# fluggo/Canvas

Hardware: AMD Instinct MI355X
Metric: Mpixels/s through 4K f16 RGBA colour-matrix+alpha-over chain; % HBM roofline (higher is better)
Workload: dtype f32

## Files before the change

### canvas_amd/_lib.py

```python
import ctypes as C
import os

from .abi import (box2i, fir_filter, rational, rgba_frame_f16, rgba_frame_f32, v2f, video_frame_source_funcs,
                  video_source)

_HERE = os.path.dirname(os.path.abspath(__file__))
LIB_PATH = os.path.join(_HERE, "libcanvas_hip.so")

CHAIN_MAX_LAYERS = 8
DISPLAY_RGBA8, DISPLAY_ARGB32_PREMUL = 0, 1
FIR_PATH_AUTO, FIR_PATH_PASSES, FIR_PATH_TILED, FIR_PATH_TABLES, FIR_PATH_HV, FIR_PATH_ONE_COLUMN, FIR_PATH_TWO_COLUMNS, FIR_PATH_STRIPS, FIR_PATH_TILES = 0, 1, 2, 4, 16, 32, 64, 128, 256
FIR_KERNEL_NONE, FIR_KERNEL_WINDOW, FIR_KERNEL_HALVE, _FIR_KERNEL_RETIRED_3, FIR_KERNEL_VH, FIR_KERNEL_TILED, _FIR_KERNEL_RETIRED_6, FIR_KERNEL_TWO_PASS, FIR_KERNEL_PASS, FIR_KERNEL_HV, FIR_KERNEL_WINDOW_PAIR, FIR_KERNEL_HALVE_PAIR, FIR_KERNEL_TILE_VH, FIR_KERNEL_UNSHARP = range(14)
ARITH_SEPARATE, ARITH_CONTRACTED = 0, 1
LUT_NONE, LUT_REC709_TO_LINEAR_SCENE, LUT_REC709_TO_LINEAR_DISPLAY, LUT_LINEAR_TO_REC709, LUT_LINEAR_TO_SRGB = -1, 0, 1, 2, 3
KEY_SHOW_MATTE = 1
YCC_PROGRESSIVE, YCC_REC709 = 1, 2


class rgba_f32(C.Structure):
    _fields_ = [("r", C.c_float), ("g", C.c_float), ("b", C.c_float), ("a", C.c_float)]


class rgba_frame_dev(C.Structure):
    _fields_ = [("data", C.c_void_p), ("format", C.c_int), ("full_window", box2i), ("current_window", box2i),
                ("stream", C.c_void_p)]


class chain_job(C.Structure):
    _fields_ = [("out", C.POINTER(rgba_frame_f16)), ("layers", C.POINTER(rgba_frame_f16) * CHAIN_MAX_LAYERS),
                ("nlayers", C.c_int)]


class chroma_key(C.Structure):
    _fields_ = [("key", C.c_float * 3), ("tolerance", C.c_float), ("softness", C.c_float), ("spill", C.c_float),
                ("spill_range", C.c_float), ("flags", C.c_int)]


class coded_image(C.Structure):
    _fields_ = [("data", C.c_void_p * 4), ("stride", C.c_int * 4), ("line_count", C.c_int * 4), ("free_func", C.c_void_p)]


P = C.POINTER
rgba_frame_f16_t = rgba_frame_f16
rgba_frame_f32_t = rgba_frame_f32
_u16p, _f32p, _vp = P(C.c_uint16), P(C.c_float), C.c_void_p
_F16, _F32 = P(rgba_frame_f16), P(rgba_frame_f32)

SIGNATURES = {
    "init_half": (None, []),
    "get_frame_time": (C.c_int64, [P(rational), C.c_int]),
    "get_time_frame": (C.c_int, [P(rational), C.c_int64]),
    "gettime": (C.c_int64, []),
    "video_get_frame_f16": (None, [P(video_source), C.c_int, _F16]),
    "video_get_frame_f32": (None, [P(video_source), C.c_int, _F32]),
    "video_get_frame_f16_gl": (None, [P(video_source), C.c_int, _F16]),
    "video_get_frame_f32_gl": (None, [P(video_source), C.c_int, _F32]),
    "video_get_frame_dev": (None, [P(video_source), C.c_int, P(rgba_frame_dev)]),
    "video_copy_frame_f16": (None, [_F16, _F16]),
    "video_copy_frame_alpha_f32": (None, [_F32, _F32, C.c_float]),
    "video_attenuate_f32": (None, [_F32, C.c_float]),
    "cvs_pulldown23_frames": (C.c_int, [C.c_int, C.c_int, P(C.c_int), P(C.c_int)]),
    "cvs_weave_fields_f16_dev": (C.c_int, [_F16, _F16, _vp]),
    "cvs_field_to_frame_f16_dev": (C.c_int, [_F16, _F16, C.c_int, _vp]),
    "cvs_soften_fields_f16_dev": (C.c_int, [_F16, _F16, _vp]),
    "cvs_interlace_fields_f16_dev": (C.c_int, [_F16, _F16, _F16, _vp]),
    "cvs_pulldown23_add_frames": (C.c_int, [C.c_int, C.c_int, P(C.c_int), P(C.c_int)]),
    "video_mix_cross_f32": (None, [_F32, _F32, _F32, C.c_float]),
    "video_mix_cross_f32_pull": (None, [_F32, P(video_source), C.c_int, P(video_source), C.c_int, C.c_float]),
    "video_mix_over_f32": (None, [_F32, _F32, C.c_float]),
    "video_scale_bilinear_f32": (None, [_F32, v2f, _F32, v2f, v2f]),
    "video_scale_bilinear_f32_pull": (None, [_F32, v2f, P(video_source), C.c_int, P(box2i), v2f, v2f]),
    "video_transfer_rec709_to_linear_scene": (None, [_u16p, _u16p, C.c_size_t]),
    "video_transfer_rec709_to_linear_display": (None, [_u16p, _u16p, C.c_size_t]),
    "video_transfer_linear_to_rec709": (None, [_u16p, _u16p, C.c_size_t]),
    "video_transfer_linear_to_sRGB": (None, [_u16p, _u16p, C.c_size_t]),
    "video_get_gamma45_ramp": (P(C.c_uint8), []),
    "video_color_rgb_to_xyz_sdtv": (None, [_F16]),
    "video_color_xyz_to_srgb": (None, [_F16]),
    "filter_createTriangle": (None, [C.c_float, C.c_float, P(fir_filter)]),
    "filter_createLanczos": (None, [C.c_float, C.c_int, C.c_float, P(fir_filter)]),
    "filter_free": (None, [P(fir_filter)]),
    "video_filter_gain_offset_f16": (None, [_F16, _F16, C.c_float, C.c_float]),
    "video_fill_solid_f16": (None, [_F16, P(box2i), P(rgba_f32)]),
    "video_fill_solid_f32": (None, [_F32, P(box2i), P(rgba_f32)]),
    "workspace_create": (_vp, []),
    "workspace_get_length": (C.c_int, [_vp]),
    "workspace_add_item": (_vp, [_vp, _vp, C.c_int64, C.c_int64, C.c_int64, C.c_int64, _vp]),
    "workspace_get_item": (_vp, [_vp, C.c_int]),
    "workspace_remove_item": (None, [_vp]),
    "workspace_as_video_source": (None, [_vp, P(video_source)]),
    "workspace_free": (None, [_vp]),
    "workspace_get_item_pos": (None, [_vp, P(C.c_int64), P(C.c_int64), P(C.c_int64)]),
    "workspace_get_item_offset": (C.c_int64, [_vp]),
    "workspace_set_item_offset": (None, [_vp, C.c_int64]),
    "workspace_get_item_source": (_vp, [_vp]),
    "workspace_set_item_source": (None, [_vp, _vp]),
    "workspace_get_item_tag": (_vp, [_vp]),
    "workspace_set_item_tag": (None, [_vp, _vp]),
    "workspace_update_item": (None, [_vp, P(C.c_int64), P(C.c_int64), P(C.c_int64), P(C.c_int64), P(_vp), P(_vp)]),
    "cvs_set_arithmetic": (C.c_int, [C.c_int]),
    "cvs_get_arithmetic": (C.c_int, []),
    "cvs_init": (C.c_int, [C.c_int]),
    "cvs_device_count": (C.c_int, []),
    "cvs_current_device": (C.c_int, []),
    "cvs_context_open": (C.c_int, [C.c_int]),
    "cvs_context_count": (C.c_int, []),
    "cvs_context_device": (C.c_int, [C.c_int]),
    "cvs_set_context": (C.c_int, [C.c_int]),
    "cvs_current_context": (C.c_int, []),
    "cvs_frame_owner": (C.c_int, [C.c_int64, C.c_int]),
    "cvs_last_error": (C.c_char_p, []),
    "cvs_clear_last_error": (None, []),
    "cvs_set_log_handler": (None, [C.c_void_p, C.c_void_p]),
    "cvs_device_name": (C.c_char_p, []),
    "cvs_compute_units": (C.c_int, []),
    "cvs_malloc": (_vp, [C.c_size_t]),
    "cvs_free": (None, [_vp]),
    "cvs_graph_begin": (C.c_int, [_vp]),
    "cvs_graph_end": (_vp, [_vp]),
    "cvs_graph_launch": (C.c_int, [_vp, _vp]),
    "cvs_graph_destroy": (None, [_vp]),
    "cvs_mem_info": (C.c_int, [P(C.c_size_t), P(C.c_size_t)]),
    "cvs_pool_malloc": (_vp, [C.c_size_t, _vp]),
    "cvs_pool_free": (None, [_vp, _vp]),
    "cvs_pool_trim": (None, []),
    "cvs_memcpy_h2d": (C.c_int, [_vp, _vp, C.c_size_t, _vp]),
    "cvs_memcpy_d2h": (C.c_int, [_vp, _vp, C.c_size_t, _vp]),
    "cvs_memcpy_d2d": (C.c_int, [_vp, _vp, C.c_size_t, _vp]),
    "cvs_memset": (C.c_int, [_vp, C.c_int, C.c_size_t, _vp]),
    "cvs_stream_create": (_vp, []),
    "cvs_stream_destroy": (None, [_vp]),
    "cvs_stream_sync": (C.c_int, [_vp]),
    "cvs_event_create": (_vp, []),
    "cvs_event_destroy": (None, [_vp]),
    "cvs_event_record": (C.c_int, [_vp, _vp]),
    "cvs_event_sync": (C.c_int, [_vp]),
    "cvs_event_elapsed_ms": (C.c_float, [_vp, _vp]),
    "cvs_lut_device": (_vp, [C.c_int]),
    "cvs_lut_host": (_u16p, [C.c_int]),
    "cvs_lut_install": (C.c_int, [C.c_int, _u16p]),
    "cvs_half_to_float_dev": (C.c_int, [_vp, _vp, C.c_size_t, _vp]),
    "cvs_float_to_half_dev": (C.c_int, [_vp, _vp, C.c_size_t, _vp]),
    "cvs_half_to_float_fast_dev": (C.c_int, [_vp, _vp, C.c_size_t, _vp]),
    "cvs_float_to_half_fast_dev": (C.c_int, [_vp, _vp, C.c_size_t, _vp]),
    "cvs_half_lookup_dev": (C.c_int, [_vp, _vp, _vp, C.c_size_t, _vp]),
    "cvs_frame_f16_to_f32_dev": (C.c_int, [_F32, _F16, _vp]),
    "cvs_frame_f32_to_f16_dev": (C.c_int, [_F16, _F32, _vp]),
    "cvs_copy_frame_f16_dev": (C.c_int, [_F16, _F16, _vp]),
    "cvs_copy_frame_alpha_f32_dev": (C.c_int, [_F32, _F32, C.c_float, _vp]),
    "cvs_mix_cross_f32_dev": (C.c_int, [_F32, _F32, _F32, C.c_float, _vp]),
    "cvs_mix_over_f32_dev": (C.c_int, [_F32, _F32, C.c_float, _vp]),
    "cvs_color_matrix_f16_dev": (C.c_int, [_F16, _f32p, C.c_int, C.c_int, _vp]),
    "cvs_color_matrix_f16_to_dev": (C.c_int, [_F16, _F16, _f32p, C.c_int, C.c_int, _vp]),
    "cvs_gain_offset_f16_dev": (C.c_int, [_F16, _F16, C.c_float, C.c_float, _vp]),
    "cvs_fill_solid_f16_dev": (C.c_int, [_F16, P(box2i), P(rgba_f32), _vp]),
    "cvs_fill_solid_f32_dev": (C.c_int, [_F32, P(box2i), P(rgba_f32), _vp]),
    "cvs_scale_bilinear_f16_dev": (C.c_int, [_F16, v2f, _F16, v2f, v2f, _vp]),
    "cvs_scale_bilinear_f32_dev": (C.c_int, [_F32, v2f, _F32, v2f, v2f, _vp]),
    "cvs_fir_blur_f32_dev": (C.c_int, [_F32, _F32, _f32p, C.c_int, _vp]),
    "coded_image_alloc": (P(coded_image), [P(C.c_int), P(C.c_int), C.c_int]),
    "coded_image_alloc0": (P(coded_image), [P(C.c_int), P(C.c_int), C.c_int]),
    "video_reconstruct_dv": (None, [_F16, P(coded_image)]),
    "video_subsample_dv": (P(coded_image), [_F16]),
    "cvs_reconstruct_dv_dev": (C.c_int, [_F16, P(coded_image), _vp]),
    "cvs_subsample_dv_dev": (C.c_int, [P(coded_image), _F16, C.c_int, _vp]),
    "video_subsample_mpeg2": (P(coded_image), [_F16]),
    "cvs_subsample_mpeg2_dev": (C.c_int, [P(coded_image), _F16, C.c_int, C.c_int, _vp]),
    "video_reconstruct_mpeg2": (None, [_F16, P(coded_image)]),
    "cvs_reconstruct_mpeg2_dev": (C.c_int, [_F16, P(coded_image), C.c_int, C.c_int, C.c_int, _vp]),
    "cvs_frame_to_bytes_dev": (C.c_int, [_vp, _F16, C.c_int, C.c_int, _vp]),
    "video_frame_to_bytes": (C.c_int, [_vp, _F16, C.c_int, C.c_int]),
    "cvs_frame_to_rgba8_intent_dev": (C.c_int, [_vp, _F16, C.c_int, C.c_float, _vp]),
    "video_frame_to_rgba8_intent": (C.c_int, [_vp, _F16, C.c_int, C.c_float]),
    "cvs_fir_blur_f16_dev": (C.c_int, [_F16, _F16, _f32p, C.c_int, _vp]),
    "cvs_unsharp_mask_f32_dev": (C.c_int, [_F32, _F32, _f32p, C.c_int, C.c_float, C.c_float, _vp]),
    "cvs_unsharp_mask_f16_dev": (C.c_int, [_F16, _F16, _f32p, C.c_int, C.c_float, C.c_float, _vp]),
    "cvs_chroma_key_f32_dev": (C.c_int, [_F32, _F32, P(chroma_key), _vp]),
    "cvs_chroma_key_f16_dev": (C.c_int, [_F16, _F16, P(chroma_key), _vp]),
    "cvs_blur_over_f16_dev": (C.c_int, [_F16, _F16, _f32p, C.c_int, P(_F16), C.c_int, _vp]),
    "cvs_resample_lanczos_f32_dev": (C.c_int, [_F32, _F32, C.c_float, C.c_float, C.c_int, _vp]),
    "cvs_resample_lanczos_f16_dev": (C.c_int, [_F16, _F16, C.c_float, C.c_float, C.c_int, _vp]),
    "cvs_blur_lanczos_f16_dev": (C.c_int, [_F16, _F16, _f32p, C.c_int, C.c_float, C.c_float, C.c_int, _vp]),
    "cvs_blur_over_f16_batch_dev": (C.c_int, [P(_F16), P(_F16), _f32p, C.c_int, P(_F16), C.c_int, C.c_int, _vp]),
    "cvs_scale_bilinear_f16_batch_dev": (C.c_int, [P(_F16), v2f, P(_F16), v2f, v2f, C.c_int, _vp]),
    "cvs_scale_bilinear_f32_batch_dev": (C.c_int, [P(_F32), v2f, P(_F32), v2f, v2f, C.c_int, _vp]),
    "cvs_blur_lanczos_f16_batch_dev": (C.c_int, [P(_F16), P(_F16), C.c_int, _f32p, C.c_int, C.c_float, C.c_float, C.c_int, _vp]),
    "cvs_fir_path_override": (None, [C.c_int]),
    "cvs_chain_color_over_f16_dev": (C.c_int, [P(chain_job), C.c_int, _f32p, C.c_int, C.c_int, _vp]),
    "cvs_chain_last_was_fused": (C.c_int, []),
    "cvs_scale_last_was_fused": (C.c_int, []),
    "cvs_fir_last_kernel": (C.c_int, []),
    "cvs_fir_fell_through_count": (C.c_int, []),
    "cvs_chain_last_launch_count": (C.c_int, []),
    "cvs_mix_cross_f16_dev": (C.c_int, [_F16, _F16, _F16, C.c_float, _vp]),
}

HALF_POINTER_GLOBALS = {
    "half_convert_to_float": C.CFUNCTYPE(None, _f32p, _u16p, C.c_int),
    "half_convert_from_float": C.CFUNCTYPE(None, _u16p, _f32p, C.c_int),
    "half_convert_to_float_fast": C.CFUNCTYPE(None, _f32p, _u16p, C.c_int),
    "half_convert_from_float_fast": C.CFUNCTYPE(None, _u16p, _f32p, C.c_int),
    "half_lookup": C.CFUNCTYPE(None, _u16p, _u16p, _u16p, C.c_int),
}

_lib = None


class LibraryMissing(RuntimeError):
    pass


def load():
    global _lib
    if _lib is not None:
        return _lib
    if not os.path.exists(LIB_PATH):
        raise LibraryMissing(
            "%s not found: build it with `python -c 'import __graft_entry__ as g; g.build()'` "
            "(or make -C canvas_amd/csrc).  There is no CPU fallback." % LIB_PATH)
    lib = C.CDLL(LIB_PATH, mode=C.RTLD_GLOBAL)
    for name, (res, args) in SIGNATURES.items():
        fn = getattr(lib, name)
        fn.restype, fn.argtypes = res, args
    _lib = lib
    return lib


def half_pointer(name):
    lib = load()
    addr = C.c_void_p.in_dll(lib, name).value
    return HALF_POINTER_GLOBALS[name](addr) if addr else None


def last_error():
    return load().cvs_last_error().decode()


def check(rc, what="call"):
    if rc != 0:
        raise RuntimeError("%s failed (%d): %s" % (what, rc, last_error()))
```

### canvas_amd/csrc/host/scale.c

```c
#define _GNU_SOURCE
#include "internal.h"
#include <limits.h>
#include <math.h>
#include <stdatomic.h>

static _Atomic int g_fir_path = CVS_FIR_PATH_AUTO;

static _Thread_local int t_scale_fused;
CVS_EXPORT int cvs_scale_last_was_fused(void) { return t_scale_fused; }
static _Thread_local int t_fir_kernel;
CVS_EXPORT int cvs_fir_last_kernel(void) { return t_fir_kernel; }
static _Thread_local int t_fell_through;
CVS_EXPORT int cvs_fir_fell_through_count(void) { return t_fell_through; }
static void fir_launch_fell_through(const char *kernel, int rc) {
    (void)hipGetLastError();
    t_fell_through++;
    cvs_log_warning("%s did not launch (%s): falling back to the next FIR kernel", kernel, hipGetErrorString((hipError_t)rc));
}
CVS_EXPORT void cvs_fir_path_override(int mode) { atomic_store(&g_fir_path, mode & (CVS_FIR_PATH_PASSES | CVS_FIR_PATH_TILED | CVS_FIR_PATH_TABLES | CVS_FIR_PATH_HV | CVS_FIR_PATH_ONE_COLUMN | CVS_FIR_PATH_TWO_COLUMNS | CVS_FIR_PATH_STRIPS | CVS_FIR_PATH_TILES)); }

typedef struct { void *data; box2i full, cur; int half; } any_frame;

static size_t any_bytes(const any_frame *f) { return cvs_box_pixels(&f->full) * (f->half ? sizeof(rgba_f16) : sizeof(rgba_f32)); }

typedef struct { void *frame, *data; box2i *full, *cur; } frame_ref;

static frame_ref frame_of(const void *f, int half) {
    frame_ref r = { (void *)f, NULL, NULL, NULL };
    if (f && half) { rgba_frame_f16 *h = r.frame; r.data = h->data; r.full = &h->full_window; r.cur = &h->current_window; }
    else if (f)    { rgba_frame_f32 *g = r.frame; r.data = g->data; r.full = &g->full_window; r.cur = &g->current_window; }
    return r;
}

static frame_ref frame_at(const void *frames, int i, int half) {
    return frame_of(half ? (const void *)((const rgba_frame_f16 *const *)frames)[i] : (const void *)((const rgba_frame_f32 *const *)frames)[i], half);
}

static any_frame any_of(const frame_ref *f, int half) {
    const any_frame a = { f->data, *f->full, *f->cur, half };
    return a;
}

static bool entry_refused(void *target, const void *source, int half, const char *what, frame_ref *t, frame_ref *src) {
    *t = frame_of(target, half);
    *src = frame_of(source, half);
    if (cvs_enter() != 0) { box2i_set_empty(t->cur); return true; }
    if (!cvs_box_contains(src->full, src->cur)) {
        cvs_set_error("%s: the input's current_window lies outside its buffer", what);
        box2i_set_empty(t->cur);
        return true;
    }
    return false;
}

static void batch_empty_from(const void *targets, int from, int count, int half) {
    for (int i = from; i < count; i++) box2i_set_empty(frame_at(targets, i, half).cur);
}

static bool batch_refused(const void *targets, const void *sources, int count, int half, const char *what) {
    if (!targets || !sources) { cvs_set_error("%s: bad arguments", what); return true; }
    for (int i = 0; i < count; i++)
        if (!frame_at(targets, i, half).frame || !frame_at(sources, i, half).frame) {
            cvs_set_error("%s: frame %d of %d is a null pointer", what, i, count);
            return true;
        }
    for (int i = 0; i < count; i++) {
        const frame_ref src = frame_at(sources, i, half);
        if (!cvs_box_contains(src.full, src.cur)) {
            cvs_set_error("%s: the input's current_window lies outside its buffer (frame %d)", what, i);
            batch_empty_from(targets, 0, count, half);
            return true;
        }
    }
    if (cvs_enter() != 0) { batch_empty_from(targets, 0, count, half); return true; }
    return false;
}

static bool same_box(const box2i *a, const box2i *b) { return memcmp(a, b, sizeof *a) == 0; }

static bool batch_group(cvk_frame_batch *b, const void *targets, const void *sources, int half, int first, int n, size_t tbytes, size_t sbytes,
                        const rgba_frame_f16 *const *overlays, int noverlays) {
    const void *in[CVK_FRAME_BATCH * (1 + CVK_BLUR_MAX_OVER)];
    int nin = 0;
    memset(b, 0, sizeof *b);
    b->n = n;
    for (int i = 0; i < n; i++) {
        b->target[i] = frame_at(targets, first + i, half).data;
        in[nin++] = b->source[i] = frame_at(sources, first + i, half).data;
        for (int l = 0; l < noverlays; l++) in[nin++] = b->over[i][l] = overlays[(size_t)(first + i) * noverlays + l]->data;
    }
    if (n < 2) return false;
    for (int i = 0; i < n; i++) {
        const char *o = b->target[i];
        for (int j = 0; j < nin; j++) { const char *q = in[j]; if (q && o < q + sbytes && q < o + tbytes) return false; }
        for (int j = 0; j < i; j++) { const char *q = b->target[j]; if (o < q + tbytes && q < o + tbytes) return false; }
    }
    return true;
}

static int gather_pass(const any_frame *t, const any_frame *src, const cvk_fir_axis *tab, int axis, int t0, int t1, int lo, int hi, hipStream_t s) {
    if (t1 < t0 || hi < lo) return 0;
    cvk_fir_params fp;
    memset(&fp, 0, sizeof fp);
    fp.target = cvs_view(t->data, &t->full);
    fp.source = cvs_view(src->data, &src->full);
    fp.axis = axis;
    fp.t0 = t0; fp.t1 = t1; fp.lo = lo; fp.hi = hi;
    fp.ntaps = tab->ntaps; fp.tap_src = tab->src; fp.taps = tab->taps; fp.stride = tab->stride;
    fp.in_half = src->half; fp.out_half = t->half;
    return CVK(cvk_fir_gather)(&fp, s);
}

static cvk_fir2d_params fir2d_params(const any_frame *t, const any_frame *src, int tx0, int ty0, int tx1, int ty1,
                                     const cvs_fir_table *h, const cvs_fir_table *v) {
    cvk_fir2d_params fp;
    memset(&fp, 0, sizeof fp);
    fp.target = cvs_view(t->data, &t->full);
    fp.source = cvs_view(src->data, &src->full);
    fp.in_half = src->half; fp.out_half = t->half;
    fp.tx0 = tx0; fp.ty0 = ty0; fp.tx1 = tx1; fp.ty1 = ty1;
    fp.h = h->axis; fp.v = v->axis;
    fp.max_sw = h->max_foot > 0 ? h->max_foot : 1;
    return fp;
}


static int triangle_pass(any_frame *target, float tmin, const any_frame *source, float smin, float factor, int axis, hipStream_t s) {
    const box2i srect = source->cur, trect = target->full;
    const int lo = axis ? (srect.min.y > trect.min.y ? srect.min.y : trect.min.y) : (srect.min.x > trect.min.x ? srect.min.x : trect.min.x);
    const int hi = axis ? (srect.max.y < trect.max.y ? srect.max.y : trect.max.y) : (srect.max.x < trect.max.x ? srect.max.x : trect.max.x);
    const int s0 = axis ? srect.min.x : srect.min.y, s1 = axis ? srect.max.x : srect.max.y;
    const int t0 = axis ? trect.min.x : trect.min.y, t1 = axis ? trect.max.x : trect.max.y;

    cvs_fir_table table;
    int rc = cvs_fir_table_triangle(tmin, smin, factor, s0, s1, t0, t1, axis == 0 || lo <= hi, &table);
    if (rc != 0) return rc;
    const int used_lo = table.used_lo, used_hi = table.used_hi;
    {
        const int o0 = axis ? trect.min.y : trect.min.x, o1 = axis ? trect.max.y : trect.max.x;
        const bool covers = used_hi >= used_lo && hi >= lo && used_lo == t0 && used_hi == t1 && lo == o0 && hi == o1;
        if (!covers && any_bytes(target)) {
            hipError_t e_ = hipMemsetAsync(target->data, 0, any_bytes(target), s);
            if (e_ != hipSuccess) { cvs_fir_table_release(&table, s); cvs_set_error("zero fill: %s", hipGetErrorString(e_)); return -1; }
        }
    }
    if (used_hi >= used_lo && hi >= lo) {
        const size_t first = (size_t)(used_lo - t0);
        cvk_fir_axis from = table.axis;
        from.ntaps += first; from.src += first * (size_t)from.stride; from.taps += first * (size_t)from.stride;
        rc = gather_pass(target, source, &from, axis, used_lo, used_hi, lo, hi, s);
        if (rc == 0) t_fir_kernel = CVS_FIR_KERNEL_PASS;
    }
    cvs_fir_table_release(&table, s);
    if (rc != 0) { cvs_set_error("FIR gather launch failed: %s", hipGetErrorString((hipError_t)rc)); return rc; }
    if (axis) box2i_set(&target->cur, used_lo, lo, used_hi, hi);
    else      box2i_set(&target->cur, lo, used_lo, hi, used_hi);
    return 0;
}

static int triangle_fused_vh(any_frame *target, v2f tp, const any_frame *source, v2f sp, v2f fac, const box2i *mid_full,
                             const cvk_frame_batch *batch, hipStream_t s) {
    const box2i *tf = &target->full, *sc = &source->cur;
    const int lo1 = sc->min.x > mid_full->min.x ? sc->min.x : mid_full->min.x, hi1 = sc->max.x < mid_full->max.x ? sc->max.x : mid_full->max.x;
    cvs_fir_table tv, th = { .pin = -1 };
    if (hi1 < lo1) return 1;
    if (cvs_fir_table_triangle(tp.y, sp.y, fac.y, sc->min.y, sc->max.y, mid_full->min.y, mid_full->max.y, true, &tv) != 0) return -1;
    const int vlo = tv.used_lo, vhi = tv.used_hi;
    int rc = 1;
    if (vhi >= vlo) {
        const int lo2 = vlo > tf->min.y ? vlo : tf->min.y, hi2 = vhi < tf->max.y ? vhi : tf->max.y;
        if (hi2 >= lo2 && cvs_fir_table_triangle(tp.x, sp.x, fac.x, lo1, hi1, tf->min.x, tf->max.x, true, &th) == 0) {
            const int hlo = th.used_lo, hhi = th.used_hi;
            cvk_fir2d_params fp = fir2d_params(target, source, tf->min.x, mid_full->min.y, tf->max.x, hi2, &th, &tv);
            const int pinned = atomic_load(&g_fir_path);
            const bool tiles = hhi >= hlo && !(pinned & CVS_FIR_PATH_STRIPS) &&
                               ((pinned & CVS_FIR_PATH_TILES) ? CVK(cvk_fir_tvh_supported)(&fp)
                                : batch && target->half ? false : CVK(cvk_fir_tvh_preferred)(&fp));
            if (batch && !(hhi >= hlo && (tiles || CVK(cvk_fir_vh_supported)(&fp)))) rc = 2;
            else if (hhi >= hlo && (tiles || CVK(cvk_fir_vh_supported)(&fp))) {
                const bool covers = lo2 == tf->min.y && hi2 == tf->max.y;
                hipError_t e = hipSuccess;
                if (batch) {
                    fp.nframes = batch->n;
                    for (int i = 0; i < batch->n; i++) {
                        fp.frame_source[i] = batch->source[i]; fp.frame_target[i] = batch->target[i];
                        if (!covers && any_bytes(target) && e == hipSuccess) e = hipMemsetAsync(batch->target[i], 0, any_bytes(target), s);
                    }
                } else if (!covers && any_bytes(target)) e = hipMemsetAsync(target->data, 0, any_bytes(target), s);
                int krc = e != hipSuccess ? (int)e : tiles ? CVK(cvk_fir_tvh)(&fp, lo2 - fp.ty0, s) : CVK(cvk_fir_vh)(&fp, lo2 - fp.ty0, cvs_cus(), s);
                if (krc == 0) { box2i_set(&target->cur, hlo, lo2, hhi, hi2); t_fir_kernel = tiles ? CVS_FIR_KERNEL_TILE_VH : CVS_FIR_KERNEL_VH; rc = 0; }
                else { fir_launch_fell_through(tiles ? "k_fir_tile_vh" : "k_fir_vh", krc); rc = 1; }
            }
        }
    }
    cvs_fir_table_release(&tv, s); cvs_fir_table_release(&th, s);
    return rc;
}

static int triangle_fused_hv(any_frame *target, v2f tp, const any_frame *source, v2f sp, v2f fac, const box2i *mid_full, hipStream_t s) {
    const box2i *tf = &target->full, *sc = &source->cur;
    const int lo1 = sc->min.y > mid_full->min.y ? sc->min.y : mid_full->min.y, hi1 = sc->max.y < mid_full->max.y ? sc->max.y : mid_full->max.y;
    cvs_fir_table th, tv = { .pin = -1 };
    if (hi1 < lo1) return 1;
    if (cvs_arith() != CVS_ARITH_SEPARATE) return 1;
    if (cvs_fir_table_triangle(tp.x, sp.x, fac.x, sc->min.x, sc->max.x, mid_full->min.x, mid_full->max.x, true, &th) != 0) return -1;
    const int hlo = th.used_lo, hhi = th.used_hi;
    int rc = 1;
    if (hhi >= hlo) {
        const int lo2 = hlo > tf->min.x ? hlo : tf->min.x, hi2 = hhi < tf->max.x ? hhi : tf->max.x;
        if (hi2 >= lo2 && cvs_fir_table_triangle(tp.y, sp.y, fac.y, lo1, hi1, tf->min.y, tf->max.y, true, &tv) == 0) {
            const int vlo = tv.used_lo, vhi = tv.used_hi;
            cvk_fir2d_params fp = fir2d_params(target, source, mid_full->min.x, tf->min.y, hi2, tf->max.y, &th, &tv);
            if (vhi >= vlo && cvk_fir_hv_supported(&fp)) {
                const bool covers = fp.tx0 == tf->min.x && hi2 == tf->max.x;
                hipError_t e = covers || !any_bytes(target) ? hipSuccess : hipMemsetAsync(target->data, 0, any_bytes(target), s);
                int krc = e != hipSuccess ? (int)e : cvk_fir_hv(&fp, cvs_cus(), s);
                if (krc == 0) { box2i_set(&target->cur, lo2, vlo, hi2, vhi); t_fir_kernel = CVS_FIR_KERNEL_HV; rc = 0; }
                else { fir_launch_fell_through("k_fir_hv", krc); rc = 1; }
            }
        }
    }
    cvs_fir_table_release(&tv, s); cvs_fir_table_release(&th, s);
    return rc;
}

static int scale_core(any_frame *target, v2f tp, const any_frame *source, v2f sp, v2f fac, const cvk_frame_batch *batch, hipStream_t s) {
    t_scale_fused = 0;
    t_fir_kernel = CVS_FIR_KERNEL_NONE;
    if (batch && ((fac.x == 1.0f && tp.x == sp.x) || (fac.y == 1.0f && tp.y == sp.y) || fac.x < fac.y ||
                  (atomic_load(&g_fir_path) & (CVS_FIR_PATH_PASSES | CVS_FIR_PATH_TILED)))) return 2;
    if (fac.x == 1.0f && tp.x == sp.x) return triangle_pass(target, tp.y, source, sp.y, fac.y, 0, s);
    if (fac.y == 1.0f && tp.y == sp.y) return triangle_pass(target, tp.x, source, sp.x, fac.x, 1, s);

    any_frame mid;
    memset(&mid, 0, sizeof mid);
    const box2i *tf = &target->full, *sc = &source->cur;
    const bool x_first = fac.x < fac.y;
    const int fl = cvs_arith() == CVS_ARITH_CONTRACTED;
    if (x_first)
        box2i_set(&mid.full, (int)madd_as(fl, -(tp.x - tf->min.x), fac.x, sp.x), sc->min.y,
                  (int)madd_as(fl, tf->max.x - tp.x, fac.x, sp.x), sc->max.y);
    else
        box2i_set(&mid.full, sc->min.x, (int)madd_as(fl, -(tp.y - tf->min.y), fac.y, sp.y),
                  sc->max.x, (int)madd_as(fl, tf->max.y - tp.y, fac.y, sp.y));
    box2i_intersect(&mid.full, &mid.full, tf);
    mid.cur = mid.full;
    if (!(atomic_load(&g_fir_path) & (CVS_FIR_PATH_PASSES | CVS_FIR_PATH_TILED))) {
        int rc = x_first ? triangle_fused_hv(target, tp, source, sp, fac, &mid.full, s) : triangle_fused_vh(target, tp, source, sp, fac, &mid.full, batch, s);
        if (rc == 0) t_scale_fused = 1;
        if (rc <= 0) return rc;
        if (batch) return 2;
    }
    size_t n = cvs_box_pixels(&mid.full);
    mid.data = cvs_pool_malloc(sizeof(rgba_f32) * (n ? n : 1), s);
    if (!mid.data) return -1;
    int rc;
    if (x_first) { rc = triangle_pass(&mid, tp.x, source, sp.x, fac.x, 1, s); if (rc == 0) rc = triangle_pass(target, tp.y, &mid, sp.y, fac.y, 0, s); }
    else         { rc = triangle_pass(&mid, tp.y, source, sp.y, fac.y, 0, s); if (rc == 0) rc = triangle_pass(target, tp.x, &mid, sp.x, fac.x, 1, s); }
    cvs_pool_free(mid.data, s);
    return rc;
}

static int scale_frame(void *target, v2f tp, const void *source, v2f sp, v2f fac, int half, cvs_stream_t stream, const char *what) {
    frame_ref t, src;
    if (entry_refused(target, source, half, what, &t, &src)) return -1;
    hipStream_t s = cvs_pick_stream(stream);
    if (fac.x == 1.0f && tp.x == sp.x && fac.y == 1.0f && tp.y == sp.y)
        return half ? cvs_copy_frame_f16_dev(target, source, s) : cvs_copy_frame_alpha_f32_dev(target, source, 1.0f, s);
    any_frame tf = any_of(&t, half);
    const any_frame sf = any_of(&src, half);
    int rc = scale_core(&tf, tp, &sf, sp, fac, NULL, s);
    *t.cur = tf.cur;
    if (rc != 0) box2i_set_empty(t.cur);
    return rc;
}

CVS_EXPORT int cvs_scale_bilinear_f32_dev(rgba_frame_f32 *target, v2f tp, const rgba_frame_f32 *source, v2f sp, v2f fac, cvs_stream_t stream) {
    return scale_frame(target, tp, source, sp, fac, 0, stream, "cvs_scale_bilinear_f32_dev");
}

CVS_EXPORT int cvs_scale_bilinear_f16_dev(rgba_frame_f16 *target, v2f tp, const rgba_frame_f16 *source, v2f sp, v2f fac, cvs_stream_t stream) {
    return scale_frame(target, tp, source, sp, fac, 1, stream, "cvs_scale_bilinear_f16_dev");
}

static int scale_batch_frames(const void *targets, v2f tp, const void *sources, v2f sp, v2f fac, int count, int half,
                              cvs_stream_t stream, const char *what) {
    if (count <= 0) return 0;
    if (batch_refused(targets, sources, count, half, what)) return -1;
    hipStream_t s = cvs_pick_stream(stream);
    const size_t px = half ? sizeof(rgba_f16) : sizeof(rgba_f32);
    int rc = 0, done = 0;
    for (int base = 0; count > 1 && rc == 0 && done == base && base < count; base += 64) {
        const int end = count - base < 64 ? count : base + 64;
        const frame_ref t0 = frame_at(targets, base, half), s0 = frame_at(sources, base, half);
        bool uniform = end - base > 1 && !box2i_is_empty(s0.cur) && !box2i_is_empty(t0.full) &&
                       !(fac.x == 1.0f && tp.x == sp.x && fac.y == 1.0f && tp.y == sp.y);
        for (int i = base + 1; uniform && i < end; i++) {
            const frame_ref ti = frame_at(targets, i, half), si = frame_at(sources, i, half);
            uniform = same_box(ti.full, t0.full) && same_box(si.full, s0.full) && same_box(si.cur, s0.cur);
        }
        const size_t tbytes = cvs_box_pixels(t0.full) * px, sbytes = cvs_box_pixels(s0.full) * px;
        while (uniform && rc == 0 && done < end) {
            const int n = end - done < CVK_FRAME_BATCH ? end - done : CVK_FRAME_BATCH;
            cvk_frame_batch b;
            if (!batch_group(&b, targets, sources, half, done, n, tbytes, sbytes, NULL, 0)) break;
            const frame_ref td = frame_at(targets, done, half), sd = frame_at(sources, done, half);
            any_frame t = any_of(&td, half);
            const any_frame src = any_of(&sd, half);
            rc = scale_core(&t, tp, &src, sp, fac, &b, s);
            if (rc == 2) { rc = 0; break; }
            if (rc != 0) break;
            for (int i = 0; i < n; i++) *frame_at(targets, done + i, half).cur = t.cur;
            done += n;
        }
    }
    for (; rc == 0 && done < count; done++) {
        void *t = frame_at(targets, done, half).frame;
        const void *src = frame_at(sources, done, half).frame;
        rc = half ? cvs_scale_bilinear_f16_dev(t, tp, src, sp, fac, stream) : cvs_scale_bilinear_f32_dev(t, tp, src, sp, fac, stream);
    }
    if (rc != 0) batch_empty_from(targets, done, count, half);
    return rc;
}

CVS_EXPORT int cvs_scale_bilinear_f16_batch_dev(rgba_frame_f16 *const *targets, v2f tp, const rgba_frame_f16 *const *sources, v2f sp, v2f fac, int count, cvs_stream_t stream) {
    return scale_batch_frames(targets, tp, sources, sp, fac, count, 1, stream, "cvs_scale_bilinear_f16_batch_dev");
}

CVS_EXPORT int cvs_scale_bilinear_f32_batch_dev(rgba_frame_f32 *const *targets, v2f tp, const rgba_frame_f32 *const *sources, v2f sp, v2f fac, int count, cvs_stream_t stream) {
    return scale_batch_frames(targets, tp, sources, sp, fac, count, 0, stream, "cvs_scale_bilinear_f32_batch_dev");
}

CVS_EXPORT void video_scale_bilinear_f32(rgba_frame_f32 *target, v2f tp, rgba_frame_f32 *source, v2f sp, v2f fac) {
    cvs_bridge br;
    rgba_frame_f32 ft, fs;
    cvs_bridge_open(&br);
    CVS_BRIDGE_FRAME(&br, ft, target, CVS_BRIDGE_UPLOAD);
    CVS_BRIDGE_FRAME(&br, fs, source, CVS_BRIDGE_PRIVATE | (box2i_is_empty(&source->current_window) ? 0 : CVS_BRIDGE_UPLOAD));
    CVS_BRIDGE_CALL(&br, cvs_scale_bilinear_f32_dev, &ft, tp, &fs, sp, fac);
    target->current_window = ft.current_window;
    if (cvs_bridge_close(&br, target->data) != 0) box2i_set_empty(&target->current_window);
}

CVS_EXPORT void video_scale_bilinear_f32_pull(rgba_frame_f32 *target, v2f tp, video_source *source, int frame,
                                              box2i *source_rect, v2f sp, v2f fac) {
    if (fac.x == 0.0f || fac.y == 0.0f) { box2i_set_empty(&target->current_window); return; }
    if (fac.x == 1.0f && fac.y == 1.0f && tp.x == sp.x && tp.y == sp.y) { video_get_frame_f32(source, frame, target); return; }
    const box2i *tf = &target->full_window;
    rgba_frame_f32 tmp;
    box2i_set(&tmp.full_window,
              (int)(sp.x - (tp.x - tf->min.x) / fac.x) - 1, (int)(sp.y - (tp.y - tf->min.y) / fac.y) - 1,
              (int)(sp.x + (tf->max.x - tp.x) / fac.x) + 1, (int)(sp.y + (tf->max.y - tp.y) / fac.y) + 1);
    box2i_intersect(&tmp.full_window, &tmp.full_window, source_rect);
    tmp.current_window = tmp.full_window;
    size_t n = cvs_box_pixels(&tmp.full_window);
    tmp.data = malloc(sizeof(rgba_f32) * (n ? n : 1));
    if (!tmp.data) { box2i_set_empty(&target->current_window); return; }
    video_get_frame_f32(source, frame, &tmp);
    video_scale_bilinear_f32(target, tp, &tmp, sp, fac);
    free(tmp.data);
}


static int fir_two_launches(const any_frame *t, const any_frame *src, const box2i *rect, const cvk_fir_axis *h, const cvk_fir_axis *v, hipStream_t s) {
    const box2i *sw = &src->cur;
    any_frame mid = { NULL, *sw, *sw, 0 };
    box2i_set(&mid.full, rect->min.x, sw->min.y, rect->max.x, sw->max.y);
    mid.data = cvs_pool_malloc(cvs_box_pixels(&mid.full) * sizeof(rgba_f32), s);
    if (!mid.data) return -1;
    int rc = gather_pass(&mid, src, h, 1, rect->min.x, rect->max.x, sw->min.y, sw->max.y, s);
    if (rc == 0) rc = gather_pass(t, &mid, v, 0, rect->min.y, rect->max.y, rect->min.x, rect->max.x, s);
    cvs_pool_free(mid.data, s);
    if (rc != 0) { cvs_set_error("FIR gather launch failed: %s", hipGetErrorString((hipError_t)rc)); return -1; }
    t_fir_kernel = CVS_FIR_KERNEL_TWO_PASS;
    return 0;
}

static int fir2d_launch(const any_frame *t, const any_frame *src, const box2i *rect, const cvs_fir_table *h, const cvs_fir_table *v, hipStream_t s) {
    cvk_fir2d_params fp = fir2d_params(t, src, rect->min.x, rect->min.y, rect->max.x, rect->max.y, h, v);
    fp.max_sh = v->max_foot > 0 ? v->max_foot : 1;
    const int force = atomic_load(&g_fir_path);
    if (force & CVS_FIR_PATH_PASSES) return 1;
    const bool pinned = (force & (CVS_FIR_PATH_TILED | CVS_FIR_PATH_HV)) != 0;
    if (cvs_arith() == CVS_ARITH_SEPARATE && ((force & CVS_FIR_PATH_HV) || !pinned) && cvk_fir_hv_supported(&fp)) {
        int rc = cvk_fir_hv(&fp, cvs_cus(), s);
        if (rc == 0) { t_fir_kernel = CVS_FIR_KERNEL_HV; return 0; }
        fir_launch_fell_through("k_fir_hv", rc);
    }
    if (CVK(cvk_fir2d_lds_bytes)(&fp) > 150 * 1024 || h->axis.stride > 64 || v->axis.stride > 64) return 1;
    int rc = CVK(cvk_fir2d)(&fp, s);
    if (rc != 0) { cvs_set_error("fused FIR launch failed: %s", hipGetErrorString((hipError_t)rc)); return -1; }
    t_fir_kernel = CVS_FIR_KERNEL_TILED;
    return 0;
}

static int fir_pair_launch(const any_frame *t, const any_frame *src, const box2i *rect, cvs_fir_table *h, cvs_fir_table *v, hipStream_t s) {
    int rc = fir2d_launch(t, src, rect, h, v, s);
    if (rc == 1) rc = fir_two_launches(t, src, rect, &h->axis, &v->axis, s);
    cvs_fir_table_release(h, s); cvs_fir_table_release(v, s);
    return rc;
}

static int blur_column_pins(void) {
    const int pin = atomic_load(&g_fir_path);
    return (pin & CVS_FIR_PATH_ONE_COLUMN ? CVK_BLUR_ONE_COLUMN : 0) | (pin & CVS_FIR_PATH_TWO_COLUMNS ? CVK_BLUR_TWO_COLUMNS : 0);
}

static bool blur_has_fast_kernel(const float *taps, int ntaps) {
    bool finite = true;
    for (int k = 0; k < ntaps; k++) finite = finite && isfinite(taps[k]);
    return finite && CVK(cvk_blur_supported)(ntaps, 1) && !(atomic_load(&g_fir_path) & CVS_FIR_PATH_TABLES);
}

static bool halving_sweep(cvk_blur_halve_params *hp, float fx, float fy, int ksize, const float *taps, int ntaps, const any_frame *t, const any_frame *src) {
    if (fx != 0.5f || fy != 0.5f || (atomic_load(&g_fir_path) & CVS_FIR_PATH_TABLES)) return false;
    const box2i *tf = &t->full, *sw = &src->cur;
    fir_filter f = { NULL, 0, 0 };
    filter_createLanczos(0.5f, ksize, 0.0f, &f);
    bool usable = f.coeff && f.center == f.width / 2 && f.width <= 16 && ntaps <= 16 &&
                  tf->min.x > -(1 << 22) && tf->max.x < (1 << 22) && tf->min.y > -(1 << 22) && tf->max.y < (1 << 22);
    for (int k = 0; usable && k < f.width; k++) usable = isfinite(f.coeff[k]);
    for (int k = 0; usable && k < ntaps; k++) usable = isfinite(taps[k]);
    if (usable) {
        memset(hp, 0, sizeof *hp);
        hp->target = cvs_view(t->data, tf);
        hp->source = cvs_view(src->data, &src->full);
        hp->in_half = 1; hp->out_half = 1;
        hp->tx0 = tf->min.x; hp->ty0 = tf->min.y; hp->tx1 = tf->max.x; hp->ty1 = tf->max.y;
        hp->sx0 = sw->min.x; hp->sy0 = sw->min.y; hp->sx1 = sw->max.x; hp->sy1 = sw->max.y;
        hp->ntaps1 = ntaps; hp->ntaps2 = f.width;
        memcpy(hp->taps1, taps, sizeof(float) * (size_t)ntaps);
        memcpy(hp->taps2, f.coeff, sizeof(float) * (size_t)f.width);
        hp->flags = blur_column_pins();
    }
    filter_free(&f);
    return usable;
}

static int halving_launch(const cvk_blur_halve_params *hp, hipStream_t s) {
    int rc = CVK(cvk_blur_halve)(hp, cvs_cus(), s);
    if (rc != 0) { cvs_set_error("blur + halving launch failed: %s", hipGetErrorString((hipError_t)rc)); return -1; }
    t_fir_kernel = CVK(cvk_blur_halve_takes_pairs)(hp) ? CVS_FIR_KERNEL_HALVE_PAIR : CVS_FIR_KERNEL_HALVE;
    return 0;
}

static int blur_fused(const any_frame *t, const any_frame *src, const box2i *win, const float *taps, int ntaps,
                      const void *const *over, int nover, const cvk_frame_batch *batch, hipStream_t s) {
    const box2i *sw = &src->cur;
    if (blur_has_fast_kernel(taps, ntaps)) {
        cvk_blur_params bp;
        memset(&bp, 0, sizeof bp);
        bp.nover = nover;
        for (int l = 0; l < nover; l++) bp.over[l] = over[l];
        bp.target = cvs_view(t->data, &t->full);
        bp.source = cvs_view(src->data, &src->full);
        bp.in_half = src->half; bp.out_half = t->half;
        bp.tx0 = win->min.x; bp.ty0 = win->min.y; bp.tx1 = win->max.x; bp.ty1 = win->max.y;
        bp.sx0 = sw->min.x; bp.sy0 = sw->min.y; bp.sx1 = sw->max.x; bp.sy1 = sw->max.y;
        bp.ntaps = ntaps;
        memcpy(bp.taps, taps, sizeof(float) * (size_t)ntaps);
        if (batch) {
            if (!(ntaps & 1) || ntaps > 31) return 1;
            bp.batch = *batch;
        }
        bp.flags = blur_column_pins();
        int rc = CVK(cvk_blur)(&bp, cvs_cus(), s);
        if (rc != 0) { cvs_set_error("blur launch failed: %s", hipGetErrorString((hipError_t)rc)); return -1; }
        t_fir_kernel = CVK(cvk_blur_takes_pairs)(&bp) ? CVS_FIR_KERNEL_WINDOW_PAIR : CVS_FIR_KERNEL_WINDOW;
        return 0;
    }
    if (nover > 0 || batch) return 1;
    cvs_fir_table h, v;
    if (cvs_fir_table_blur(taps, ntaps, win->min.x, win->max.x, sw->min.x, sw->max.x, CVK_FIR2D_TILE_X, &h) != 0) return -1;
    if (cvs_fir_table_blur(taps, ntaps, win->min.y, win->max.y, sw->min.y, sw->max.y, CVK_FIR2D_TILE_Y, &v) != 0) { cvs_fir_table_release(&h, s); return -1; }
    return fir_pair_launch(t, src, win, &h, &v, s);
}

static int lanczos_fused(const any_frame *t, const any_frame *src, float fx, float fy, int ksize, hipStream_t s) {
    const box2i *tfull = &t->full, *sw = &src->cur;
    const float identity = 1.0f;
    cvk_blur_halve_params hp;
    if (halving_sweep(&hp, fx, fy, ksize, &identity, 1, t, src) && CVK(cvk_blur_supported)(hp.ntaps2, 2)) {
        int rc, kernel;
        if (src->half && t->half && CVK(cvk_blur_halve_takes_pairs)(&hp)) {
            rc = CVK(cvk_blur_halve_pair)(&hp, cvs_cus(), s);
            kernel = CVS_FIR_KERNEL_HALVE_PAIR;
        } else {
            cvk_blur_params bp;
            memset(&bp, 0, sizeof bp);
            bp.target = hp.target; bp.source = hp.source;
            bp.in_half = src->half; bp.out_half = t->half;
            bp.tx0 = hp.tx0; bp.ty0 = hp.ty0; bp.tx1 = hp.tx1; bp.ty1 = hp.ty1;
            bp.sx0 = hp.sx0; bp.sy0 = hp.sy0; bp.sx1 = hp.sx1; bp.sy1 = hp.sy1;
            bp.ntaps = hp.ntaps2; bp.step = 2;
            memcpy(bp.taps, hp.taps2, sizeof(float) * (size_t)hp.ntaps2);
            rc = CVK(cvk_blur)(&bp, cvs_cus(), s);
            kernel = CVS_FIR_KERNEL_WINDOW;
        }
        if (rc != 0) { cvs_set_error("resample launch failed: %s", hipGetErrorString((hipError_t)rc)); return -1; }
        t_fir_kernel = kernel;
        return 0;
    }
    cvs_fir_table h, v;
    if (cvs_fir_table_lanczos(fx, ksize, tfull->min.x, tfull->max.x, sw->min.x, sw->max.x, CVK_FIR2D_TILE_X, &h) != 0) return -1;
    if (cvs_fir_table_lanczos(fy, ksize, tfull->min.y, tfull->max.y, sw->min.y, sw->max.y, CVK_FIR2D_TILE_Y, &v) != 0) { cvs_fir_table_release(&h, s); return -1; }
    return fir_pair_launch(t, src, tfull, &h, &v, s);
}

static int fir_blur(void *target, const void *source, const float *taps, int ntaps, int half, cvs_stream_t stream, const char *what) {
    frame_ref t, src;
    if (entry_refused(target, source, half, what, &t, &src)) return -1;
    if (ntaps < 1 || !taps) { cvs_set_error("blur: need at least one tap"); box2i_set_empty(t.cur); return -1; }
    hipStream_t s = cvs_pick_stream(stream);
    box2i win;
    box2i_intersect(&win, src.cur, t.full);
    *t.cur = win;
    if (box2i_is_empty(&win)) return 0;
    const any_frame tf = any_of(&t, half), sf = any_of(&src, half);
    int rc = blur_fused(&tf, &sf, &win, taps, ntaps, NULL, 0, NULL, s);
    if (rc != 0) box2i_set_empty(t.cur);
    return rc;
}

CVS_EXPORT int cvs_fir_blur_f32_dev(rgba_frame_f32 *target, const rgba_frame_f32 *source, const float *taps, int ntaps, cvs_stream_t stream) {
    return fir_blur(target, source, taps, ntaps, 0, stream, "cvs_fir_blur_f32_dev");
}

CVS_EXPORT int cvs_fir_blur_f16_dev(rgba_frame_f16 *target, const rgba_frame_f16 *source, const float *taps, int ntaps, cvs_stream_t stream) {
    return fir_blur(target, source, taps, ntaps, 1, stream, "cvs_fir_blur_f16_dev");
}

static int unsharp_mask(void *target, const void *source, const float *taps, int ntaps, float amount, float threshold, int half,
                        cvs_stream_t stream, const char *what) {
    frame_ref t, src;
    if (entry_refused(target, source, half, what, &t, &src)) return -1;
    if (ntaps < 1 || !taps) { cvs_set_error("unsharp mask: need at least one tap"); box2i_set_empty(t.cur); return -1; }
    hipStream_t s = cvs_pick_stream(stream);
    box2i win;
    box2i_intersect(&win, src.cur, t.full);
    *t.cur = win;
    const bool fused = blur_has_fast_kernel(taps, ntaps) && CVK(cvk_unsharp_supported)(ntaps);
    t_fir_kernel = fused ? CVS_FIR_KERNEL_UNSHARP : CVS_FIR_KERNEL_NONE;
    if (box2i_is_empty(&win)) return 0;
    const any_frame tf = any_of(&t, half), sf = any_of(&src, half);
    int rc;
    if (fused) {
        cvk_unsharp_params up;
        memset(&up, 0, sizeof up);
        up.target = cvs_view(tf.data, &tf.full);
        up.source = cvs_view(sf.data, &sf.full);
        up.half = half;
        up.tx0 = win.min.x; up.ty0 = win.min.y; up.tx1 = win.max.x; up.ty1 = win.max.y;
        up.sx0 = sf.cur.min.x; up.sy0 = sf.cur.min.y; up.sx1 = sf.cur.max.x; up.sy1 = sf.cur.max.y;
        up.ntaps = ntaps;
        up.amount = amount; up.threshold = threshold;
        memcpy(up.taps, taps, sizeof(float) * (size_t)ntaps);
        rc = CVK(cvk_unsharp)(&up, cvs_cus(), s);
        if (rc != 0) { cvs_set_error("unsharp mask launch failed: %s", hipGetErrorString((hipError_t)rc)); rc = -1; }
    } else {
        any_frame mid = { NULL, win, win, 0 };
        mid.data = cvs_pool_malloc(cvs_box_pixels(&win) * sizeof(rgba_f32), s);
        if (!mid.data) { box2i_set_empty(t.cur); return -1; }
        rc = blur_fused(&mid, &sf, &win, taps, ntaps, NULL, 0, NULL, s);
        if (rc == 0) {
            const cvk_rect r = { win.min.x, win.min.y, win.max.x, win.max.y };
            rc = CVK(cvk_unsharp_combine)(cvs_view(tf.data, &tf.full), cvs_view(sf.data, &sf.full), cvs_view(mid.data, &mid.full), r, half, amount, threshold, s);
            if (rc != 0) { cvs_set_error("unsharp mask launch failed: %s", hipGetErrorString((hipError_t)rc)); rc = -1; }
        }
        cvs_pool_free(mid.data, s);
    }
    if (rc != 0) box2i_set_empty(t.cur);
    return rc;
}

CVS_EXPORT int cvs_unsharp_mask_f32_dev(rgba_frame_f32 *target, const rgba_frame_f32 *source, const float *taps, int ntaps, float amount, float threshold, cvs_stream_t s) {
    return unsharp_mask(target, source, taps, ntaps, amount, threshold, 0, s, "cvs_unsharp_mask_f32_dev");
}

CVS_EXPORT int cvs_unsharp_mask_f16_dev(rgba_frame_f16 *target, const rgba_frame_f16 *source, const float *taps, int ntaps, float amount, float threshold, cvs_stream_t s) {
    return unsharp_mask(target, source, taps, ntaps, amount, threshold, 1, s, "cvs_unsharp_mask_f16_dev");
}

CVS_EXPORT int cvs_blur_over_f16_dev(rgba_frame_f16 *out, const rgba_frame_f16 *source, const float *taps, int ntaps,
                                     const rgba_frame_f16 *const *overlays, int noverlays, cvs_stream_t stream) {
    if (cvs_enter() != 0) { box2i_set_empty(&out->current_window); return -1; }
    CVS_REQUIRE_INSIDE(source, out, "cvs_blur_over_f16_dev");
    if (ntaps < 1 || !taps || noverlays < 0 || (noverlays > 0 && !overlays)) { cvs_set_error("blur+over: bad arguments"); box2i_set_empty(&out->current_window); return -1; }
    if (noverlays == 0) return cvs_fir_blur_f16_dev(out, source, taps, ntaps, stream);
    hipStream_t s = cvs_pick_stream(stream);
    const box2i *full = &out->full_window;
    if (box2i_is_empty(full)) { box2i_set_empty(&out->current_window); return 0; }
    const any_frame o = { out->data, *full, *full, 1 }, src = { (void *)source->data, source->full_window, source->current_window, 1 };
    box2i win;
    box2i_intersect(&win, &source->current_window, full);
    bool whole = noverlays <= CVK_BLUR_MAX_OVER && memcmp(&win, full, sizeof win) == 0;
    const void *bufs[CVK_BLUR_MAX_OVER];
    for (int l = 0; whole && l < noverlays; l++) {
        whole = memcmp(&overlays[l]->full_window, full, sizeof *full) == 0 && memcmp(&overlays[l]->current_window, full, sizeof *full) == 0;
        bufs[l] = overlays[l]->data;
    }
    int rc = 1;
    if (whole && noverlays > 0) rc = blur_fused(&o, &src, &win, taps, ntaps, bufs, noverlays, NULL, s);
    if (rc == 0) { out->current_window = *full; return 0; }
    if (rc < 0) { box2i_set_empty(&out->current_window); return rc; }

    rgba_frame_f32 acc = { cvs_pool_malloc(cvs_box_pixels(full) * sizeof(rgba_f32), s), *full, *full };
    rgba_frame_f32 tmp = { noverlays > 0 ? cvs_pool_malloc(cvs_box_pixels(full) * sizeof(rgba_f32), s) : NULL, *full, *full };
    rc = (acc.data && (tmp.data || noverlays == 0)) ? 0 : -1;
    if (rc == 0) {
        box2i_set_empty(&acc.current_window);
        if (!box2i_is_empty(&win)) {
            const any_frame a = { acc.data, *full, win, 0 };
            acc.current_window = win;
            rc = blur_fused(&a, &src, &win, taps, ntaps, NULL, 0, NULL, s);
        }
    }
    for (int l = 0; rc == 0 && l < noverlays; l++) {
        rc = cvs_frame_f16_to_f32_dev(&tmp, overlays[l], s);
        if (rc == 0) rc = cvs_mix_over_f32_dev(&acc, &tmp, 1.0f, s);
    }
    if (rc == 0) rc = cvs_frame_f32_to_f16_dev(out, &acc, s);
    cvs_pool_free(acc.data, s); cvs_pool_free(tmp.data, s);
    if (rc != 0) box2i_set_empty(&out->current_window);
    return rc;
}

static int resample_lanczos(void *target, const void *source, float fx, float fy, int ksize, int half, cvs_stream_t stream, const char *what) {
    frame_ref t, src;
    if (entry_refused(target, source, half, what, &t, &src)) return -1;
    if (!(fx > 0.0f) || !(fy > 0.0f) || ksize < 1 || box2i_is_empty(src.cur) || box2i_is_empty(t.full)) {
        box2i_set_empty(t.cur);
        return 0;
    }
    hipStream_t s = cvs_pick_stream(stream);
    const any_frame tf = any_of(&t, half), sf = any_of(&src, half);
    int rc = lanczos_fused(&tf, &sf, fx, fy, ksize, s);
    if (rc == 0) *t.cur = *t.full;
    else box2i_set_empty(t.cur);
    return rc;
}

CVS_EXPORT int cvs_resample_lanczos_f32_dev(rgba_frame_f32 *target, const rgba_frame_f32 *source, float fx, float fy, int ksize, cvs_stream_t stream) {
    return resample_lanczos(target, source, fx, fy, ksize, 0, stream, "cvs_resample_lanczos_f32_dev");
}

CVS_EXPORT int cvs_resample_lanczos_f16_dev(rgba_frame_f16 *target, const rgba_frame_f16 *source, float fx, float fy, int ksize, cvs_stream_t stream) {
    return resample_lanczos(target, source, fx, fy, ksize, 1, stream, "cvs_resample_lanczos_f16_dev");
}

CVS_EXPORT int cvs_blur_lanczos_f16_dev(rgba_frame_f16 *target, const rgba_frame_f16 *source, const float *taps, int ntaps,
                                        float fx, float fy, int ksize, cvs_stream_t stream) {
    if (cvs_enter() != 0) { box2i_set_empty(&target->current_window); return -1; }
    CVS_REQUIRE_INSIDE(source, target, "cvs_blur_lanczos_f16_dev");
    if (ntaps < 1 || !taps || !(fx > 0.0f) || !(fy > 0.0f) || ksize < 1) { cvs_set_error("blur+lanczos: bad arguments"); box2i_set_empty(&target->current_window); return -1; }
    if (box2i_is_empty(&source->current_window) || box2i_is_empty(&target->full_window)) { box2i_set_empty(&target->current_window); return 0; }
    hipStream_t s = cvs_pick_stream(stream);
    const box2i *sw = &source->current_window;
    const any_frame tf = { target->data, target->full_window, target->full_window, 1 }, sf = { (void *)source->data, source->full_window, *sw, 1 };
    if (ntaps == 1 && taps[0] == 1.0f) return cvs_resample_lanczos_f16_dev(target, source, fx, fy, ksize, stream);
    cvk_blur_halve_params hp;
    if ((ntaps & 1) && halving_sweep(&hp, fx, fy, ksize, taps, ntaps, &tf, &sf) && CVK(cvk_blur_halve_supported)(ntaps, hp.ntaps2)) {
        const int rc = halving_launch(&hp, s);
        if (rc == 0) target->current_window = target->full_window;
        else box2i_set_empty(&target->current_window);
        return rc;
    }
    any_frame mid = { NULL, *sw, *sw, 0 };
    mid.data = cvs_pool_malloc(cvs_box_pixels(sw) * sizeof(rgba_f32), s);
    if (!mid.data) { box2i_set_empty(&target->current_window); return -1; }
    int rc = blur_fused(&mid, &sf, sw, taps, ntaps, NULL, 0, NULL, s);
    if (rc == 0) rc = lanczos_fused(&tf, &mid, fx, fy, ksize, s);
    if (rc == 0) target->current_window = target->full_window;
    cvs_pool_free(mid.data, s);
    if (rc != 0) box2i_set_empty(&target->current_window);
    return rc;
}

CVS_EXPORT int cvs_blur_over_f16_batch_dev(rgba_frame_f16 *const *outs, const rgba_frame_f16 *const *sources, const float *taps, int ntaps,
                                           const rgba_frame_f16 *const *overlays, int noverlays, int count, cvs_stream_t stream) {
    const char *what = "cvs_blur_over_f16_batch_dev";
    if (count <= 0) return 0;
    if (ntaps < 1 || !taps || noverlays < 0 || (noverlays > 0 && !overlays)) { cvs_set_error("%s: bad arguments", what); return -1; }
    for (int i = 0; i < count; i++)
        for (int l = 0; l < noverlays; l++)
            if (!overlays[(size_t)i * noverlays + l]) { cvs_set_error("%s: layer %d of frame %d is a null pointer", what, l, i); return -1; }
    if (batch_refused(outs, sources, count, 1, what)) return -1;
    hipStream_t s = cvs_pick_stream(stream);
    const box2i *full = &outs[0]->full_window;
    bool uniform = count > 1 && noverlays >= 1 && noverlays <= CVK_BLUR_MAX_OVER && !box2i_is_empty(full) && blur_has_fast_kernel(taps, ntaps) && (ntaps & 1);
    for (int i = 0; uniform && i < count; i++) {
        uniform = same_box(&outs[i]->full_window, full) && same_box(&sources[i]->full_window, &sources[0]->full_window) &&
                  same_box(&sources[i]->current_window, full) && same_box(&sources[0]->full_window, full);
        for (int l = 0; uniform && l < noverlays; l++) {
            const rgba_frame_f16 *ov = overlays[(size_t)i * noverlays + l];
            uniform = same_box(&ov->full_window, full) && same_box(&ov->current_window, full);
        }
    }
    int rc = 0, done = 0;
    const size_t bytes = cvs_box_pixels(full) * sizeof(rgba_f16);
    while (uniform && rc == 0 && done < count) {
        const int n = count - done < CVK_FRAME_BATCH ? count - done : CVK_FRAME_BATCH;
        cvk_frame_batch b;
        if (!batch_group(&b, outs, sources, 1, done, n, bytes, bytes, overlays, noverlays)) break;
        const any_frame t = { b.target[0], *full, *full, 1 }, src = { (void *)b.source[0], sources[done]->full_window, sources[done]->current_window, 1 };
        rc = blur_fused(&t, &src, full, taps, ntaps, b.over[0], noverlays, &b, s);
        if (rc == 1) { rc = 0; break; }
        if (rc == 0) { for (int i = 0; i < n; i++) outs[done + i]->current_window = *full; done += n; }
    }
    for (; rc == 0 && done < count; done++)
        rc = cvs_blur_over_f16_dev(outs[done], sources[done], taps, ntaps, noverlays ? overlays + (size_t)done * noverlays : NULL, noverlays, stream);
    if (rc != 0) batch_empty_from(outs, done, count, 1);
    return rc;
}

CVS_EXPORT int cvs_blur_lanczos_f16_batch_dev(rgba_frame_f16 *const *targets, const rgba_frame_f16 *const *sources, int count,
                                              const float *taps, int ntaps, float fx, float fy, int ksize, cvs_stream_t stream) {
    const char *what = "cvs_blur_lanczos_f16_batch_dev";
    if (count <= 0) return 0;
    if (ntaps < 1 || !taps || !(fx > 0.0f) || !(fy > 0.0f) || ksize < 1) { cvs_set_error("%s: bad arguments", what); return -1; }
    if (batch_refused(targets, sources, count, 1, what)) return -1;
    hipStream_t s = cvs_pick_stream(stream);
    int rc = 0, done = 0;
    const box2i *tf = &targets[0]->full_window, *sw = &sources[0]->current_window;
    bool uniform = count > 1 && (ntaps & 1) && !(ntaps == 1 && taps[0] == 1.0f) && !box2i_is_empty(sw) && !box2i_is_empty(tf);
    for (int i = 1; uniform && i < count; i++)
        uniform = same_box(&targets[i]->full_window, tf) && same_box(&sources[i]->full_window, &sources[0]->full_window) &&
                  same_box(&sources[i]->current_window, sw);
    const any_frame t0 = { targets[0]->data, *tf, *tf, 1 }, s0 = { (void *)sources[0]->data, sources[0]->full_window, *sw, 1 };
    cvk_blur_halve_params hp;
    if (uniform && halving_sweep(&hp, fx, fy, ksize, taps, ntaps, &t0, &s0) && CVK(cvk_blur_halve_supported)(ntaps, hp.ntaps2)) {
        const size_t sbytes = cvs_box_pixels(&sources[0]->full_window) * sizeof(rgba_f16), tbytes = cvs_box_pixels(tf) * sizeof(rgba_f16);
        while (rc == 0 && done < count) {
            const int n = count - done < CVK_FRAME_BATCH ? count - done : CVK_FRAME_BATCH;
            if (!batch_group(&hp.batch, targets, sources, 1, done, n, tbytes, sbytes, NULL, 0)) break;
            hp.target.data = hp.batch.target[0];
            hp.source.data = (void *)hp.batch.source[0];
            if ((rc = halving_launch(&hp, s)) != 0) break;
            for (int i = 0; i < n; i++) targets[done + i]->current_window = targets[done + i]->full_window;
            done += n;
        }
    }
    for (; rc == 0 && done < count; done++)
        rc = cvs_blur_lanczos_f16_dev(targets[done], sources[done], taps, ntaps, fx, fy, ksize, stream);
    if (rc != 0) batch_empty_from(targets, done, count, 1);
    return rc;
}
```

### canvas_amd/csrc/kernels/blur_pair_ops.hip

```cpp
#include <cstdlib>
#include <atomic>
#include "pair_common.hpp"

namespace {

using namespace pairsweep;

template <int NT, int W, int NOV>
__global__ __launch_bounds__(W) void k_blur_pair(cvk_blur_params bp) {
    constexpr int C = NT / 2, D = C & 1, OUTW = 2 * W - 2 * C - 2 * D, PITCH = W + 8;
    static_assert(NT & 1 && NT >= 3 && NT <= 15, "odd tap counts up to 15");
    static_assert(NOV >= 0 && NOV <= CVK_BLUR_MAX_OVER, "layer count");
    __shared__ float4 rowbuf[2][2][PITCH];
    const int lane = threadIdx.x;
    const int xo = bp.tx0 + (int)blockIdx.x * OUTW;
    const int sfirst = xo - C - D;
    const int tcol = xo + 2 * lane;
    const int ta = bp.ty0 + (int)blockIdx.y * bp.rows_per_wg;
    const int tb = min(ta + bp.rows_per_wg - 1, bp.ty1);
    const int ys0 = ta - C;
    const int steps = (tb - ta) + NT;

    float w[NT];
#pragma unroll
    for (int k = 0; k < NT; k++) w[k] = bp.taps[k];

    const int z = (int)blockIdx.z;
    typedef const cvk_blur_params __attribute__((address_space(4))) *kargs_t;
    const kargs_t ka = (kargs_t)__builtin_amdgcn_kernarg_segment_ptr();
    const void *src_data = bp.batch.n ? ka->batch.source[z] : bp.source.data;
    void *dst_data = bp.batch.n ? ka->batch.target[z] : bp.target.data;
    const void *over_data[NOV > 0 ? NOV : 1];
#pragma unroll
    for (int l = 0; l < NOV; l++) over_data[l] = bp.batch.n ? ka->batch.over[z][l] : bp.over[l];

    const size_t srow = (size_t)bp.source.pitch * 8, trow = (size_t)bp.target.pitch * 8;
    const uint32_t soff = (uint32_t)((sfirst + 2 * lane - bp.sx0) * 8);
    const uint32_t toff = 2 * lane < OUTW ? (uint32_t)((tcol - bp.tx0) * 8) : 0x80000000u;
#ifdef CVS_DIAG
    const uint32_t swin = (bp.flags & 0x100) ? 0u : (uint32_t)(bp.sx1 - bp.sx0 + 1) * 8u, trect = (uint32_t)(bp.tx1 - bp.tx0 + 1) * 8u;
    const uint32_t orect = (bp.flags & 0x200) ? 0u : trect, wrect = (bp.flags & 0x400) ? 0u : trect;
#else
    const uint32_t swin = (uint32_t)(bp.sx1 - bp.sx0 + 1) * 8u, trect = (uint32_t)(bp.tx1 - bp.tx0 + 1) * 8u, orect = trect, wrect = trect;
#endif
    const char *swin0 = reinterpret_cast<const char *>(src_data) + (ptrdiff_t)(bp.sx0 - bp.source.fx0) * 8;
    const ptrdiff_t trect0 = (ptrdiff_t)(bp.tx0 - bp.target.fx0) * 8;

    if (lane < PITCH - W) {
#pragma unroll
        for (int b = 0; b < 2; b++)
#pragma unroll
            for (int ph = 0; ph < 2; ph++) rowbuf[b][ph][W + lane] = make_float4(0.f, 0.f, 0.f, 0.f);
    }

    Px ring[NT][2];
#pragma unroll
    for (int k = 0; k < NT; k++) ring[k][0].rg = ring[k][0].ba = ring[k][1].rg = ring[k][1].ba = f32x2{ 0.0f, 0.0f };

    auto fetch_row = [&](int ys, bool wanted) {
        const bool live = wanted && ys >= bp.sy0 && ys <= bp.sy1;
        return load_pair(row_rsrc(swin0, (size_t)((ptrdiff_t)(ys - bp.source.fy0) * (ptrdiff_t)srow), live ? swin : 0u), soff);
    };
    struct Layers { u32x4 v[NOV > 0 ? NOV : 1]; };
    auto fetch_layers = [&](int i) {
        Layers r;
        const bool emits = i >= NT - 1 && i < steps;
        const size_t o = (size_t)((ptrdiff_t)(ta + i - (NT - 1) - bp.target.fy0) * (ptrdiff_t)trow + trect0);
#pragma unroll
        for (int l = 0; l < NOV; l++) r.v[l] = load_pair(row_rsrc(over_data[l], o, emits ? orect : 0u), toff);
        return r;
    };
    u32x4 cur = fetch_row(ys0, true);
    rowbuf[0][0][lane] = widen_px(cur.x, cur.y);
    rowbuf[0][1][lane] = widen_px(cur.z, cur.w);
    cur = fetch_row(ys0 + 1, steps > 1);
    u32x4 nxt = fetch_row(ys0 + 2, steps > 2);
    Layers ov_cur = fetch_layers(0);

    for (int i0 = 0; i0 < steps; i0 += NT) {
        auto step = [&](auto jc) -> bool {
            constexpr int j = decltype(jc)::value;
            const int i = i0 + j;
            if (i >= steps) return false;
            const bool emits = i >= NT - 1;
            const int t = ta + (i - (NT - 1));
            const u32x4 far = fetch_row(ys0 + i + 3, i + 3 < steps);
            const Layers ov_nxt = fetch_layers(i + 1);
            float4 (*buf)[PITCH] = rowbuf[i & 1];
            __syncthreads();
            float4 v[NT + 1];
#pragma unroll
            for (int c = 0; c <= NT; c++) v[c] = buf[(c + D) & 1][lane + ((c + D) >> 1)];
            float4 (*nbuf)[PITCH] = rowbuf[(i + 1) & 1];
            nbuf[0][lane] = widen_px(cur.x, cur.y);
            nbuf[1][lane] = widen_px(cur.z, cur.w);
            cur = nxt;
            nxt = far;
            f32x2 rg0, ba0, rg1, ba1;
#pragma unroll
            for (int k = 0; k < NT; k++) {
                if constexpr (cvs::kContract) {
                    if (k == 0) { rg0 = f32x2{ v[0].x, v[0].y } * w[0]; ba0 = f32x2{ v[0].z, v[0].w } * w[0]; rg1 = f32x2{ v[1].x, v[1].y } * w[0]; ba1 = f32x2{ v[1].z, v[1].w } * w[0]; }
                    else {
                        rg0 = cvs::madd(f32x2{ v[k].x, v[k].y }, w[k], rg0); ba0 = cvs::madd(f32x2{ v[k].z, v[k].w }, w[k], ba0);
                        rg1 = cvs::madd(f32x2{ v[k + 1].x, v[k + 1].y }, w[k], rg1); ba1 = cvs::madd(f32x2{ v[k + 1].z, v[k + 1].w }, w[k], ba1);
                    }
                } else {
                const f32x2 p0 = f32x2{ v[k].x, v[k].y } * w[k], q0 = f32x2{ v[k].z, v[k].w } * w[k];
                const f32x2 p1 = f32x2{ v[k + 1].x, v[k + 1].y } * w[k], q1 = f32x2{ v[k + 1].z, v[k + 1].w } * w[k];
                if (k == 0) { rg0 = p0; ba0 = q0; rg1 = p1; ba1 = q1; }
                else { rg0 = rg0 + p0; ba0 = ba0 + q0; rg1 = rg1 + p1; ba1 = ba1 + q1; }
                }
            }
            ring[j][0].rg = rg0; ring[j][0].ba = ba0;
            ring[j][1].rg = rg1; ring[j][1].ba = ba1;
            if (emits) {
                f32x2 org0, oba0, org1, oba1;
#pragma unroll
                for (int k = 0; k < NT; k++) {
                    const Px &a = ring[(j + 1 + k) % NT][0], &b = ring[(j + 1 + k) % NT][1];
                    if constexpr (cvs::kContract) {
                        if (k == 0) { org0 = a.rg * w[0]; oba0 = a.ba * w[0]; org1 = b.rg * w[0]; oba1 = b.ba * w[0]; }
                        else { org0 = cvs::madd(a.rg, w[k], org0); oba0 = cvs::madd(a.ba, w[k], oba0); org1 = cvs::madd(b.rg, w[k], org1); oba1 = cvs::madd(b.ba, w[k], oba1); }
                    } else {
                    const f32x2 p0 = a.rg * w[k], q0 = a.ba * w[k], p1 = b.rg * w[k], q1 = b.ba * w[k];
                    if (k == 0) { org0 = p0; oba0 = q0; org1 = p1; oba1 = q1; }
                    else { org0 = org0 + p0; oba0 = oba0 + q0; org1 = org1 + p1; oba1 = oba1 + q1; }
                    }
                }
                u32x4 codes;
                if constexpr (NOV > 0) {
                    cvs::px32x2 acc;
                    acc.r = f32x2{ org0.x, org1.x }; acc.g = f32x2{ org0.y, org1.y };
                    acc.b = f32x2{ oba0.x, oba1.x }; acc.a = f32x2{ oba0.y, oba1.y };
#pragma unroll
                    for (int l = 0; l < NOV; l++) acc = cvs::over_pair_uniform(acc, ov_cur.v[l]);
                    codes = cvs::narrow_pair_lean(acc);
                } else {
                    codes = u32x4{ cvs::f2h_rz2(org0.x, org0.y), cvs::f2h_rz2(oba0.x, oba0.y), cvs::f2h_rz2(org1.x, org1.y), cvs::f2h_rz2(oba1.x, oba1.y) };
                }
                __builtin_amdgcn_raw_buffer_store_b128(codes, row_rsrc(dst_data, (size_t)((ptrdiff_t)(t - bp.target.fy0) * (ptrdiff_t)trow + trect0), wrect), (int)toff, 0, 0);
            }
            ov_cur = ov_nxt;
            return true;
        };
        each_slot(step, std::make_integer_sequence<int, NT>{});
    }
}

template <int NT, int W, int NOV>
int launch(cvk_blur_params bp, int cus, hipStream_t s) {
    constexpr int C = NT / 2, D = C & 1, OUTW = 2 * W - 2 * C - 2 * D;
    const int cols = bp.tx1 - bp.tx0 + 1, rows = bp.ty1 - bp.ty0 + 1;
    const int strips = (cols + OUTW - 1) / OUTW;
    static std::atomic<int> cached{ 0 };
    int mine = cached.load(std::memory_order_relaxed);
    if (!mine) {
        mine = resident_per_cu(k_blur_pair<NT, W, NOV>, W);
        const char *e = CVS_DIAG_ENV("CVS_BLUR_PAIR_WGS");
        if (e && atoi(e) > 0) mine = atoi(e);
        cached.store(mine, std::memory_order_relaxed);
    }
    const int nframes = bp.batch.n > 0 ? bp.batch.n : 1;
    if (bp.rows_per_wg <= 0) {
        int segs = (mine * cus) / (strips * nframes);
        if (segs < 1) segs = 1;
        int r = (rows + segs - 1) / segs;
        if (r < NT - 1) r = NT - 1;
        if (r > rows) r = rows;
        bp.rows_per_wg = r;
    }
    dim3 grid((unsigned)strips, (unsigned)((rows + bp.rows_per_wg - 1) / bp.rows_per_wg), (unsigned)nframes);
    hipLaunchKernelGGL((k_blur_pair<NT, W, NOV>), grid, dim3(W), 0, s, bp);
    return (int)hipGetLastError();
}

template <int NT, int W>
int pick_layers(const cvk_blur_params *bp, int cus, hipStream_t s) {
    switch (bp->nover) {
    case 0: return launch<NT, W, 0>(*bp, cus, s);
    case 1: return launch<NT, W, 1>(*bp, cus, s);
    case 2: return launch<NT, W, 2>(*bp, cus, s);
    case 3: return launch<NT, W, 3>(*bp, cus, s);
    case 4: return launch<NT, W, 4>(*bp, cus, s);
    }
    return (int)hipErrorInvalidValue;
}

template <int W>
int pick(const cvk_blur_params *bp, int cus, hipStream_t s) {
    switch (bp->ntaps) {
    case 3: return pick_layers<3, W>(bp, cus, s);
    case 5: return pick_layers<5, W>(bp, cus, s);
    case 7: return pick_layers<7, W>(bp, cus, s);
    case 9: return pick_layers<9, W>(bp, cus, s);
    case 11: return pick_layers<11, W>(bp, cus, s);
    case 13: return pick_layers<13, W>(bp, cus, s);
    }
    return (int)hipErrorInvalidValue;
}

}

extern "C" int cvk_blur_pair_supported(const cvk_blur_params *bp) {
    if (!(bp->in_half && bp->out_half) || (bp->step != 0 && bp->step != 1)) return 0;
    if (!(bp->ntaps & 1) || bp->ntaps < 3 || bp->ntaps > 13) return 0;
    if (bp->nover < 0 || bp->nover > CVK_BLUR_MAX_OVER) return 0;
    const int c = bp->ntaps / 2, d = c & 1;
    if ((bp->source.pitch | bp->target.pitch) & 1) return 0;
    if (((bp->tx0 - bp->target.fx0) | (bp->tx1 - bp->tx0 + 1)) & 1) return 0;
    if (((bp->sx0 - bp->source.fx0) | (bp->sx1 - bp->sx0 + 1) | (bp->tx0 - c - d - bp->sx0)) & 1) return 0;
    if (bp->sx1 < bp->sx0 || bp->sy1 < bp->sy0) return 0;
    const int n = bp->batch.n > 0 ? bp->batch.n : 1;
    if (n > CVK_FRAME_BATCH) return 0;
    for (int z = 0; z < n; z++) {
        const void *src = bp->batch.n ? bp->batch.source[z] : bp->source.data;
        const void *dst = bp->batch.n ? bp->batch.target[z] : bp->target.data;
        if (!aligned16(src) || !aligned16(dst)) return 0;
        for (int l = 0; l < bp->nover; l++)
            if (!aligned16(bp->batch.n ? bp->batch.over[z][l] : bp->over[l])) return 0;
    }
    return 1;
}

extern "C" int cvk_blur_pair(const cvk_blur_params *bp_in, int cus, void *stream) {
    if (bp_in->tx1 < bp_in->tx0 || bp_in->ty1 < bp_in->ty0) return 0;
    if (!cvk_blur_pair_supported(bp_in)) return (int)hipErrorInvalidValue;
    cvk_blur_params bp = *bp_in;
    bp.step = 1;
    bp.flags = 0;
#ifdef CVS_DIAG
    { const char *e = getenv("CVS_BLUR_PAIR_DROP"); if (e) bp.flags = atoi(e) << 8; }
#endif
    return pick<64>(&bp, cus, (hipStream_t)stream);
}
```

### canvas_amd/csrc/kernels/kernels.h

```cpp
#ifndef CVS_KERNELS_H
#define CVS_KERNELS_H

#include <stddef.h>
#include <stdint.h>

#ifdef CVS_DIAG
#include <stdlib.h>
#define CVS_DIAG_ENV(name) getenv(name)
#else
#define CVS_DIAG_ENV(name) ((const char *)0)
#endif

#ifdef CVS_CONTRACT
#define cvk_gain_offset_f16          cvk_gain_offset_f16_fma
#define cvk_mix                      cvk_mix_fma
#define cvk_color_matrix             cvk_color_matrix_fma
#define cvk_chain_color_over         cvk_chain_color_over_fma
#define cvk_chain_cross              cvk_chain_cross_fma
#define cvk_chain_count_reset        cvk_chain_count_reset_fma
#define cvk_chain_count              cvk_chain_count_fma
#define cvk_fir_gather               cvk_fir_gather_fma
#define cvk_fir2d_lds_bytes          cvk_fir2d_lds_bytes_fma
#define cvk_fir2d                    cvk_fir2d_fma
#define cvk_fir_vh_supported         cvk_fir_vh_supported_fma
#define cvk_fir_vh                   cvk_fir_vh_fma
#define cvk_fir_tvh_supported        cvk_fir_tvh_supported_fma
#define cvk_fir_tvh_preferred        cvk_fir_tvh_preferred_fma
#define cvk_fir_tvh                  cvk_fir_tvh_fma
#define cvk_blur_supported           cvk_blur_supported_fma
#define cvk_blur_takes_pairs         cvk_blur_takes_pairs_fma
#define cvk_blur                     cvk_blur_fma
#define cvk_blur_pair_supported      cvk_blur_pair_supported_fma
#define cvk_blur_pair                cvk_blur_pair_fma
#define cvk_blur_halve_pair_supported cvk_blur_halve_pair_supported_fma
#define cvk_blur_halve_pair          cvk_blur_halve_pair_fma
#define cvk_blur_halve_supported     cvk_blur_halve_supported_fma
#define cvk_blur_halve_takes_pairs   cvk_blur_halve_takes_pairs_fma
#define cvk_blur_halve               cvk_blur_halve_fma
#define cvk_unsharp_supported        cvk_unsharp_supported_fma
#define cvk_unsharp                  cvk_unsharp_fma
#define cvk_unsharp_combine          cvk_unsharp_combine_fma
#define cvk_dv_reconstruct           cvk_dv_reconstruct_fma
#define cvk_dv_subsample             cvk_dv_subsample_fma
#endif

#ifdef __cplusplus
extern "C" {
#endif

typedef struct {
    void *data;
    int pitch;
    int fx0, fy0, fx1, fy1;
} cvk_view;

typedef struct { int x0, y0, x1, y1; } cvk_rect;

int cvk_half_to_float(float *out, const uint16_t *in, size_t count, int fast, void *stream);
int cvk_float_to_half(uint16_t *out, const float *in, size_t count, int fast, void *stream);
int cvk_half_lookup(const uint16_t *table, uint16_t *out, const uint16_t *in, size_t count, int cus, void *stream);

int cvk_copy_f16(cvk_view out, cvk_view in, cvk_rect r, void *stream);
int cvk_copy_alpha_f32(cvk_view out, cvk_view in, cvk_rect r, float alpha, void *stream);
int cvk_weave_f16(cvk_view frame, cvk_rect cur, const void *other, cvk_rect other_cur, void *stream);
int cvk_widen(cvk_view out32, cvk_view in16, cvk_rect r, void *stream);
int cvk_narrow(cvk_view out16, cvk_view in32, cvk_rect r, void *stream);
int cvk_fill_f16(cvk_view out, cvk_rect r, const float rgba[4], void *stream);
int cvk_fill_f32(cvk_view out, cvk_rect r, const float rgba[4], void *stream);
int cvk_gain_offset_f16(cvk_view out, cvk_view in, cvk_rect r, float gain, float offset, void *stream);

enum { CVK_MIX_CROSS = 0, CVK_MIX_OVER = 1 };
typedef struct {
    cvk_view out, p, q;
    cvk_rect outer, inner;
    cvk_rect pw, qw;
    int gap_x, gap_y;
    int top_is_p, bottom_is_p, left_is_p, right_is_p;
    float wp, wq;
    int mode;
    int p_in_place;
} cvk_mix_params;
int cvk_mix(const cvk_mix_params *mp, void *stream);

int cvk_color_matrix(cvk_view dst, cvk_view src, cvk_rect r, const float m[9], const uint16_t *pre_lut,
                     const uint16_t *post_lut, int cus, void *stream);

#define CVK_CHAIN_MAX_LAYERS 8
typedef struct {
    void *out;
    const void *layer[CVK_CHAIN_MAX_LAYERS];
    int nlayers;
    int pad;
    uint64_t npixels;
} cvk_chain_job;
int cvk_chain_color_over(const cvk_chain_job *jobs, int njobs, int uniform_layers, const float *m,
                         const uint16_t *pre_lut, const uint16_t *post_lut, int cus, void *stream);

void cvk_chain_count_reset(void);
int cvk_chain_count(void);

int cvk_chain_cross(const cvk_chain_job *jobs, int njobs, float wa, float wb, int cus, void *stream);

typedef struct {
    cvk_view target, source;
    int axis;
    int t0, t1;
    int lo, hi;
    int s0, s1;
    const int *ntaps;
    const int *tap_src;
    const float *taps;
    int stride;
    int in_half, out_half;
} cvk_fir_params;
int cvk_fir_gather(const cvk_fir_params *fp, void *stream);
int cvk_zero_f32(cvk_view v, void *stream);

typedef struct {
    const int *ntaps, *src;
    const float *taps;
    const int *foot;
    int stride;
    int lines;
    int max_taps;
    int wide_foot;
    int max_active;
    int streamable;
    const uint32_t *lrec;
    const uint32_t *pack;
    int pack_width;
    int span_lines[3];
} cvk_fir_axis;
#define CVK_FIR_LREC 32
#define CVK_AXIS_ALIGN(bytes)              (((size_t)(bytes) + 255) & ~(size_t)255)
#define CVK_AXIS_NLINES(lines)             ((size_t)((lines) > 0 ? (lines) : 1))
#define CVK_AXIS_OFF_SRC(lines)            CVK_AXIS_ALIGN(CVK_AXIS_NLINES(lines) * 4)
#define CVK_AXIS_OFF_TAPS(lines, stride)   (CVK_AXIS_OFF_SRC(lines) + CVK_AXIS_ALIGN(CVK_AXIS_NLINES(lines) * (size_t)(stride) * 4))
#define CVK_AXIS_OFF_FOOT(lines, stride)   (CVK_AXIS_OFF_TAPS(lines, stride) + CVK_AXIS_ALIGN(CVK_AXIS_NLINES(lines) * (size_t)(stride) * 4))
#define CVK_FIR_TVH_LINES 16
typedef struct {
    cvk_view target, source;
    int in_half, out_half;
    int tx0, ty0, tx1, ty1;
    cvk_fir_axis h, v;
    int max_sw, max_sh;
    int nframes, pad_;
    const void *frame_source[8];
    void *frame_target[8];
} cvk_fir2d_params;
#define CVK_FIR2D_TILE_X 32
#define CVK_FIR2D_TILE_Y 16
int cvk_fir_hv_supported(const cvk_fir2d_params *fp);
int cvk_fir_hv(const cvk_fir2d_params *fp, int cus, void *stream);
int cvk_fir_vh_supported(const cvk_fir2d_params *fp);
int cvk_fir_vh(const cvk_fir2d_params *fp, int line0, int cus, void *stream);
int cvk_fir_tvh_supported(const cvk_fir2d_params *fp);
int cvk_fir_tvh_preferred(const cvk_fir2d_params *fp);
int cvk_fir_tvh(const cvk_fir2d_params *fp, int line0, void *stream);
size_t cvk_fir2d_lds_bytes(const cvk_fir2d_params *fp);
int cvk_fir2d(const cvk_fir2d_params *fp, void *stream);

#define CVK_FRAME_BATCH 8
#define CVK_BLUR_MAX_OVER 4
typedef struct {
    int n, pad;
    const void *source[CVK_FRAME_BATCH];
    void *target[CVK_FRAME_BATCH];
    const void *over[CVK_FRAME_BATCH][CVK_BLUR_MAX_OVER];
} cvk_frame_batch;

typedef struct {
    cvk_view target, source;
    int in_half, out_half;
    int tx0, ty0, tx1, ty1;
    int sx0, sy0, sx1, sy1;
    int ntaps;
    int rows_per_wg;
    int step;
    float taps[32];
    int nover;
    int flags;
    const void *over[CVK_BLUR_MAX_OVER];
    cvk_frame_batch batch;
} cvk_blur_params;
#define CVK_BLUR_ONE_COLUMN  1
#define CVK_BLUR_TWO_COLUMNS 2
int cvk_blur_supported(int ntaps, int step);
int cvk_blur(const cvk_blur_params *bp, int cus, void *stream);
int cvk_blur_takes_pairs(const cvk_blur_params *bp);
int cvk_blur_pair_supported(const cvk_blur_params *bp);
int cvk_blur_pair(const cvk_blur_params *bp, int cus, void *stream);

typedef struct {
    cvk_view target, source;
    int in_half, out_half;
    int tx0, ty0, tx1, ty1;
    int sx0, sy0, sx1, sy1;
    int ntaps1, ntaps2;
    int rows_per_wg;
    int flags;
    float taps1[16], taps2[16];
    cvk_frame_batch batch;
} cvk_blur_halve_params;
int cvk_blur_halve_supported(int ntaps1, int ntaps2);
int cvk_blur_halve_pair_supported(const cvk_blur_halve_params *bp);
int cvk_blur_halve_pair(const cvk_blur_halve_params *bp, int cus, void *stream);
int cvk_blur_halve_takes_pairs(const cvk_blur_halve_params *bp);
int cvk_blur_halve(const cvk_blur_halve_params *bp, int cus, void *stream);

typedef struct {
    cvk_view target, source;
    int half;
    int tx0, ty0, tx1, ty1;
    int sx0, sy0, sx1, sy1;
    int ntaps;
    int rows_per_wg;
    float amount, threshold;
    float taps[16];
} cvk_unsharp_params;
int cvk_unsharp_supported(int ntaps);
int cvk_unsharp(const cvk_unsharp_params *up, int cus, void *stream);
int cvk_unsharp_combine(cvk_view out, cvk_view src, cvk_view blurred, cvk_rect r, int half, float amount, float threshold, void *stream);

enum { CVK_DISPLAY_RGBA8 = 0, CVK_DISPLAY_ARGB32_PREMUL = 1 };
int cvk_display(void *dst, cvk_view src, cvk_rect r, const uint8_t *table, int mode, int cus, void *stream);

typedef struct { uint8_t *y, *cb, *cr; int sy, scb, scr; } cvk_dv_planes;
typedef struct { float coeff[16]; int width, center; } cvk_dv_taps;
int cvk_dv_reconstruct(cvk_view frame, cvk_rect cur, const cvk_dv_planes *pl, const cvk_dv_taps *tri, const uint16_t *lut, void *stream);
int cvk_dv_subsample(const cvk_dv_planes *pl, cvk_view frame, cvk_rect w, const cvk_dv_taps *tri, const uint16_t *lut, int encode_in_place, void *stream);

int cvk_mpeg2_subsample(const cvk_dv_planes *pl, cvk_view frame, cvk_rect w, int width, int height, const uint16_t *lut, int cus, void *stream);
int cvk_mpeg2_reconstruct(cvk_view frame, cvk_rect w, const cvk_dv_planes *pl, int width, int height, int progressive, const float mat[9],
                          const uint16_t *lut, int cus, void *stream);

int cvk_field_to_frame(cvk_view out, cvk_view in, cvk_rect w, cvk_rect in_cur, int field, int cus, void *stream);
int cvk_soften_fields(cvk_view out, cvk_view in, cvk_rect w, cvk_rect in_cur, int cus, void *stream);
int cvk_interlace_fields(cvk_view out, cvk_view even, cvk_view odd, cvk_rect w, cvk_rect even_cur, cvk_rect odd_cur, int cus, void *stream);

typedef struct {
    float kpb, kpr, tolerance, inv_soft, inv_spill, spill;
    int soft, fade;
    int matte;
} cvk_key_params;
int cvk_chroma_key(const cvk_key_params *kp, cvk_view out, cvk_view in, cvk_rect w, int half, int cus, void *stream);

#ifndef CVS_CONTRACT
int cvk_gain_offset_f16_fma(cvk_view out, cvk_view in, cvk_rect r, float gain, float offset, void *stream);
int cvk_mix_fma(const cvk_mix_params *mp, void *stream);
int cvk_color_matrix_fma(cvk_view dst, cvk_view src, cvk_rect r, const float m[9], const uint16_t *pre_lut, const uint16_t *post_lut, int cus, void *stream);
int cvk_chain_color_over_fma(const cvk_chain_job *jobs, int njobs, int uniform_layers, const float *m, const uint16_t *pre_lut, const uint16_t *post_lut, int cus, void *stream);
int cvk_chain_cross_fma(const cvk_chain_job *jobs, int njobs, float wa, float wb, int cus, void *stream);
void cvk_chain_count_reset_fma(void);
int cvk_chain_count_fma(void);
int cvk_fir_gather_fma(const cvk_fir_params *fp, void *stream);
size_t cvk_fir2d_lds_bytes_fma(const cvk_fir2d_params *fp);
int cvk_fir2d_fma(const cvk_fir2d_params *fp, void *stream);
int cvk_fir_vh_supported_fma(const cvk_fir2d_params *fp);
int cvk_fir_vh_fma(const cvk_fir2d_params *fp, int line0, int cus, void *stream);
int cvk_fir_tvh_supported_fma(const cvk_fir2d_params *fp);
int cvk_fir_tvh_preferred_fma(const cvk_fir2d_params *fp);
int cvk_fir_tvh_fma(const cvk_fir2d_params *fp, int line0, void *stream);
int cvk_blur_supported_fma(int ntaps, int step);
int cvk_blur_takes_pairs_fma(const cvk_blur_params *bp);
int cvk_blur_fma(const cvk_blur_params *bp, int cus, void *stream);
int cvk_blur_pair_supported_fma(const cvk_blur_params *bp);
int cvk_blur_pair_fma(const cvk_blur_params *bp, int cus, void *stream);
int cvk_blur_halve_pair_supported_fma(const cvk_blur_halve_params *bp);
int cvk_blur_halve_pair_fma(const cvk_blur_halve_params *bp, int cus, void *stream);
int cvk_blur_halve_supported_fma(int ntaps1, int ntaps2);
int cvk_blur_halve_takes_pairs_fma(const cvk_blur_halve_params *bp);
int cvk_blur_halve_fma(const cvk_blur_halve_params *bp, int cus, void *stream);
int cvk_unsharp_supported_fma(int ntaps);
int cvk_unsharp_fma(const cvk_unsharp_params *up, int cus, void *stream);
int cvk_unsharp_combine_fma(cvk_view out, cvk_view src, cvk_view blurred, cvk_rect r, int half, float amount, float threshold, void *stream);
int cvk_dv_reconstruct_fma(cvk_view frame, cvk_rect cur, const cvk_dv_planes *pl, const cvk_dv_taps *tri, const uint16_t *lut, void *stream);
int cvk_dv_subsample_fma(const cvk_dv_planes *pl, cvk_view frame, cvk_rect w, const cvk_dv_taps *tri, const uint16_t *lut, int encode_in_place, void *stream);
#endif

#ifdef __cplusplus
}
#endif
#endif
```

### canvas_amd/stream.py

```python
import ctypes as C

import numpy as np

from . import _lib, synth
from .device import DeviceFrame
from .shard import frames_of_rank

NODE_BYTES_PER_PIXEL = 16 + 16 + 40
BYTES_PER_PIXEL = 16 + 40
OVERLAYS = 3


class GraphStream:

    def __init__(self, width, height, ring=4, matrix=None, pre_lut=_lib.LUT_REC709_TO_LINEAR_SCENE,
                 post_lut=_lib.LUT_NONE, taps=None, overlays=OVERLAYS, first_frame=0, frame_step=1, exact_slots=None, donors=None):
        from . import REC709_RGB_TO_YPBPR
        self.lib = _lib.load()
        self.w, self.h, self.ring, self.overlays = width, height, ring, overlays
        self.full = (0, 0, width - 1, height - 1)
        self.matrix = np.ascontiguousarray(REC709_RGB_TO_YPBPR if matrix is None else matrix, np.float32).reshape(9)
        self.pre_lut, self.post_lut = pre_lut, post_lut
        self.taps = np.ascontiguousarray(synth.gaussian_taps(9, 1.5) if taps is None else taps, np.float32)
        self.slots = []
        nd = 0
        for slot in range(ring):
            exact = exact_slots is None or slot < exact_slots or not donors
            frames = []
            for k in range(overlays + 1):
                d = DeviceFrame(self.full, np.uint16)
                if exact:
                    d.upload(synth.layer_pixels(width, height, k, first_frame + slot * frame_step))
                else:
                    src_frame = donors[(2 * nd) % len(donors)] if k == 0 else donors[(2 * nd + 1) % len(donors)]
                    nd += 1
                    _lib.check(self.lib.cvs_memcpy_d2d(d.ptr, src_frame.ptr, d.nbytes, None), "d2d")
                frames.append(d)
            src, over = frames[0], frames[1:]
            refs = (C.POINTER(_lib.rgba_frame_f16_t) * overlays)(*[C.pointer(o.c) for o in over])
            self.slots.append({"src": src, "over": over, "over_refs": refs, "graded": DeviceFrame(self.full, np.uint16),
                               "out": DeviceFrame(self.full, np.uint16)})
        _lib.check(self.lib.cvs_stream_sync(None), "donor copies")
        self._m = self.matrix.ctypes.data_as(C.POINTER(C.c_float))
        self._t = self.taps.ctypes.data_as(C.POINTER(C.c_float))

    @staticmethod
    def host_inputs(width, height, frame, overlays=OVERLAYS):
        return [synth.layer_frame(width, height, k, frame) for k in range(overlays + 1)]

    def render(self, slot, stream=None):
        s, lib = self.slots[slot % self.ring], self.lib
        _lib.check(lib.cvs_color_matrix_f16_to_dev(s["graded"].ref(), s["src"].ref(), self._m, self.pre_lut, self.post_lut, stream), "colour")
        _lib.check(lib.cvs_blur_over_f16_dev(s["out"].ref(), s["graded"].ref(), self._t, len(self.taps), s["over_refs"],
                                             self.overlays, stream), "blur+over")
        return s["out"]

    def render_batch(self, slots, stream=None):
        lib, n = self.lib, len(slots)
        ss = [self.slots[i % self.ring] for i in slots]
        for s in ss:
            _lib.check(lib.cvs_color_matrix_f16_to_dev(s["graded"].ref(), s["src"].ref(), self._m, self.pre_lut, self.post_lut, stream), "colour")
        key = tuple(i % self.ring for i in slots)
        if getattr(self, "_batch_key", None) != key:
            fp = C.POINTER(_lib.rgba_frame_f16_t)
            self._b_out = (fp * n)(*[C.pointer(s["out"].c) for s in ss])
            self._b_src = (fp * n)(*[C.pointer(s["graded"].c) for s in ss])
            self._b_ov = (fp * (n * self.overlays))(*[C.pointer(o.c) for s in ss for o in s["over"]])
            self._batch_key = key
        _lib.check(lib.cvs_blur_over_f16_batch_dev(self._b_out, self._b_src, self._t, len(self.taps), self._b_ov, self.overlays, n, stream), "blur+over batch")
        return [s["out"] for s in ss]

    def run(self, frames_per_rank, rank=0, world=1, stream=None):
        mine = frames_of_rank(rank, world, frames_per_rank)
        for i, _g in enumerate(mine):
            self.render(i, stream)
        return len(mine)
```

### include/canvas_hip.h

```cpp
#ifndef CANVAS_HIP_H
#define CANVAS_HIP_H

#include <stdint.h>
#include <stddef.h>
#include <stdbool.h>

#if defined(__cplusplus)
extern "C" {
#endif

#define CVS_EXPORT __attribute__((visibility("default")))
#define NS_PER_SEC INT64_C(1000000000)


typedef uint16_t half;
#define HALF_COUNT 65536

typedef struct { int32_t n; uint32_t d; } rational;
typedef struct { int32_t x, y; } v2i;
typedef struct { v2i min, max; } box2i;
typedef struct { float x, y; } v2f;
typedef struct { v2f min, max; } box2f;

typedef struct { half r, g, b, a; } rgba_f16;
typedef struct { uint8_t r, g, b, a; } rgba_u8;
typedef struct { float r, g, b, a; } rgba_f32;

typedef struct { rgba_f16 *data; box2i full_window; box2i current_window; } rgba_frame_f16;
typedef struct { rgba_f32 *data; box2i full_window; box2i current_window; } rgba_frame_f32;

enum { CVS_FORMAT_F16 = 1, CVS_FORMAT_F32 = 2 };
typedef struct {
    void *data;
    int format;
    box2i full_window;
    box2i current_window;
    void *stream;
} rgba_frame_dev;

typedef void (*video_get_frame_func)(void *self, int frame_index, rgba_frame_f16 *frame);
typedef void (*video_get_frame_32_func)(void *self, int frame_index, rgba_frame_f32 *frame);
typedef void (*video_get_frame_dev_func)(void *self, int frame_index, rgba_frame_dev *frame);

#define VIDEO_SOURCE_FLAG_DEVICE 0x1

typedef struct {
    int flags;
    video_get_frame_func get_frame;
    video_get_frame_32_func get_frame_32;
    video_get_frame_dev_func get_frame_dev;
} video_frame_source_funcs;

typedef struct { void *obj; video_frame_source_funcs *funcs; } video_source;

typedef struct { float *coeff; int width; int center; } fir_filter;


static inline void v2i_add(v2i *r, const v2i *a, const v2i *b) { r->x = a->x + b->x; r->y = a->y + b->y; }
static inline void v2i_subtract(v2i *r, const v2i *a, const v2i *b) { r->x = a->x - b->x; r->y = a->y - b->y; }

#if !defined(__cplusplus)
static inline int min(int a, int b) { return a < b ? a : b; }
static inline int max(int a, int b) { return a > b ? a : b; }
static inline int clamp(int v, int lo, int hi) { return min(max(v, lo), hi); }
#endif
static inline float minf(float a, float b) { return a < b ? a : b; }
static inline float maxf(float a, float b) { return a > b ? a : b; }
static inline float clampf(float v, float lo, float hi) { return minf(maxf(v, lo), hi); }

static inline void box2i_set(box2i *b, int x0, int y0, int x1, int y1) { b->min.x = x0; b->min.y = y0; b->max.x = x1; b->max.y = y1; }
static inline void box2i_set_empty(box2i *b) { box2i_set(b, 0, 0, -1, -1); }
static inline bool box2i_is_empty(const box2i *b) { return b->max.x < b->min.x || b->max.y < b->min.y; }
static inline void box2i_intersect(box2i *r, const box2i *a, const box2i *b) {
    int x0 = a->min.x > b->min.x ? a->min.x : b->min.x, y0 = a->min.y > b->min.y ? a->min.y : b->min.y;
    int x1 = a->max.x < b->max.x ? a->max.x : b->max.x, y1 = a->max.y < b->max.y ? a->max.y : b->max.y;
    box2i_set(r, x0, y0, x1, y1);
}
static inline void box2i_union(box2i *r, const box2i *a, const box2i *b) {
    int x0 = a->min.x < b->min.x ? a->min.x : b->min.x, y0 = a->min.y < b->min.y ? a->min.y : b->min.y;
    int x1 = a->max.x > b->max.x ? a->max.x : b->max.x, y1 = a->max.y > b->max.y ? a->max.y : b->max.y;
    box2i_set(r, x0, y0, x1, y1);
}
static inline void box2i_normalize(box2i *b) {
    if (b->min.x > b->max.x) { int32_t t = b->min.x - 1; b->min.x = b->max.x + 1; b->max.x = t; }
    if (b->min.y > b->max.y) { int32_t t = b->min.y - 1; b->min.y = b->max.y + 1; b->max.y = t; }
}
static inline void box2i_get_size(const box2i *b, v2i *r) {
    r->x = b->max.x < b->min.x ? 0 : b->max.x - b->min.x + 1;
    r->y = b->max.y < b->min.y ? 0 : b->max.y - b->min.y + 1;
}
static inline rgba_f16 *video_get_pixel_f16(rgba_frame_f16 *f, int x, int y) {
    return &f->data[(ptrdiff_t)(y - f->full_window.min.y) * (f->full_window.max.x - f->full_window.min.x + 1) + x - f->full_window.min.x];
}
static inline rgba_f32 *video_get_pixel_f32(rgba_frame_f32 *f, int x, int y) {
    return &f->data[(ptrdiff_t)(y - f->full_window.min.y) * (f->full_window.max.x - f->full_window.min.x + 1) + x - f->full_window.min.x];
}


CVS_EXPORT void init_half(void);
CVS_EXPORT extern void (*half_convert_from_float)(half *out, const float *in, int count);
CVS_EXPORT extern void (*half_convert_to_float)(float *out, const half *in, int count);
CVS_EXPORT extern void (*half_convert_from_float_fast)(half *out, const float *in, int count);
CVS_EXPORT extern void (*half_convert_to_float_fast)(float *out, const half *in, int count);
CVS_EXPORT extern void (*half_lookup)(const half *table, half *out, const half *in, int count);

static inline void rgba_f32_to_f16(rgba_f16 *out, const rgba_f32 *in, int count) { half_convert_from_float(&out->r, &in->r, count * 4); }
static inline void rgba_f16_to_f32(rgba_f32 *out, const rgba_f16 *in, int count) { half_convert_to_float(&out->r, &in->r, count * 4); }

CVS_EXPORT int64_t get_frame_time(const rational *frame_rate, int frame);
CVS_EXPORT int get_time_frame(const rational *frame_rate, int64_t time);
CVS_EXPORT int64_t gettime(void);

CVS_EXPORT void video_get_frame_f16(video_source *source, int frame_index, rgba_frame_f16 *frame);
CVS_EXPORT void video_get_frame_f32(video_source *source, int frame_index, rgba_frame_f32 *frame);
CVS_EXPORT void video_get_frame_f16_gl(video_source *source, int frame_index, rgba_frame_f16 *frame);
CVS_EXPORT void video_get_frame_f32_gl(video_source *source, int frame_index, rgba_frame_f32 *frame);
CVS_EXPORT void video_get_frame_dev(video_source *source, int frame_index, rgba_frame_dev *frame);

CVS_EXPORT void video_copy_frame_f16(rgba_frame_f16 *out, rgba_frame_f16 *in);
CVS_EXPORT void video_copy_frame_alpha_f32(rgba_frame_f32 *out, rgba_frame_f32 *in, float alpha);
CVS_EXPORT void video_attenuate_f32(rgba_frame_f32 *frame, float alpha);
CVS_EXPORT void video_mix_cross_f32(rgba_frame_f32 *out, rgba_frame_f32 *a, rgba_frame_f32 *b, float mix_b);
CVS_EXPORT void video_mix_cross_f32_pull(rgba_frame_f32 *out, video_source *a, int frame_a, video_source *b, int frame_b, float mix_b);
CVS_EXPORT void video_mix_over_f32(rgba_frame_f32 *out, rgba_frame_f32 *b, float mix_b);

CVS_EXPORT void video_scale_bilinear_f32(rgba_frame_f32 *target, v2f target_point, rgba_frame_f32 *source, v2f source_point, v2f factors);
CVS_EXPORT void video_scale_bilinear_f32_pull(rgba_frame_f32 *target, v2f target_point, video_source *source, int frame,
                                              box2i *source_rect, v2f source_point, v2f factors);

CVS_EXPORT void video_transfer_rec709_to_linear_scene(half *out, const half *in, size_t count);
CVS_EXPORT void video_transfer_rec709_to_linear_display(half *out, const half *in, size_t count);
CVS_EXPORT void video_transfer_linear_to_rec709(half *out, const half *in, size_t count);
CVS_EXPORT void video_transfer_linear_to_sRGB(half *out, const half *in, size_t count);
CVS_EXPORT const uint8_t *video_get_gamma45_ramp(void);

CVS_EXPORT void video_color_rgb_to_xyz_sdtv(rgba_frame_f16 *frame);
CVS_EXPORT void video_color_xyz_to_srgb(rgba_frame_f16 *frame);

CVS_EXPORT void filter_createTriangle(float sub, float offset, fir_filter *filter);
CVS_EXPORT void filter_createLanczos(float sub, int kernel_size, float offset, fir_filter *filter);
CVS_EXPORT void filter_free(fir_filter *filter);

CVS_EXPORT void video_filter_gain_offset_f16(rgba_frame_f16 *out, rgba_frame_f16 *in, float gain, float offset);

CVS_EXPORT void video_fill_solid_f16(rgba_frame_f16 *frame, const box2i *window, const rgba_f32 *color);
CVS_EXPORT void video_fill_solid_f32(rgba_frame_f32 *frame, const box2i *window, const rgba_f32 *color);

typedef struct workspace_t_tag workspace_t;
typedef struct workspace_item_t_tag workspace_item_t;
CVS_EXPORT workspace_t *workspace_create(void);
CVS_EXPORT int workspace_get_length(workspace_t *workspace);
CVS_EXPORT workspace_item_t *workspace_add_item(workspace_t *self, void *source, int64_t x, int64_t width, int64_t offset, int64_t z, void *tag);
CVS_EXPORT workspace_item_t *workspace_get_item(workspace_t *self, int index);
CVS_EXPORT void workspace_remove_item(workspace_item_t *item);
CVS_EXPORT void workspace_as_video_source(workspace_t *workspace, video_source *source);
CVS_EXPORT void workspace_free(workspace_t *workspace);
CVS_EXPORT void workspace_get_item_pos(workspace_item_t *item, int64_t *x, int64_t *width, int64_t *z);
CVS_EXPORT int64_t workspace_get_item_offset(workspace_item_t *item);
CVS_EXPORT void workspace_set_item_offset(workspace_item_t *item, int64_t offset);
CVS_EXPORT void *workspace_get_item_source(workspace_item_t *item);
CVS_EXPORT void workspace_set_item_source(workspace_item_t *item, void *source);
CVS_EXPORT void *workspace_get_item_tag(workspace_item_t *item);
CVS_EXPORT void workspace_set_item_tag(workspace_item_t *item, void *tag);
CVS_EXPORT void workspace_update_item(workspace_item_t *item, int64_t *x, int64_t *width, int64_t *z, int64_t *offset, void **source, void **tag);


typedef void *cvs_stream_t;

enum { CVS_LUT_NONE = -1, CVS_LUT_REC709_TO_LINEAR_SCENE = 0, CVS_LUT_REC709_TO_LINEAR_DISPLAY = 1,
       CVS_LUT_LINEAR_TO_REC709 = 2, CVS_LUT_LINEAR_TO_SRGB = 3, CVS_LUT_COUNT = 4 };

enum { CVS_ARITH_SEPARATE = 0, CVS_ARITH_CONTRACTED = 1 };
CVS_EXPORT int cvs_set_arithmetic(int mode);
CVS_EXPORT int cvs_get_arithmetic(void);

CVS_EXPORT int cvs_init(int device);
CVS_EXPORT int cvs_device_count(void);
CVS_EXPORT int cvs_current_device(void);

CVS_EXPORT int cvs_context_open(int device);
CVS_EXPORT int cvs_context_count(void);
CVS_EXPORT int cvs_context_device(int ctx);
CVS_EXPORT int cvs_set_context(int ctx);
CVS_EXPORT int cvs_current_context(void);
CVS_EXPORT int cvs_frame_owner(int64_t frame_index, int nowners);
CVS_EXPORT const char *cvs_last_error(void);
CVS_EXPORT void cvs_clear_last_error(void);
enum { CVS_LOG_ERROR = 0, CVS_LOG_WARNING = 1, CVS_LOG_INFO = 2 };
typedef void (*cvs_log_func)(const char *domain, int level, const char *message, void *user_data);
CVS_EXPORT void cvs_set_log_handler(cvs_log_func handler, void *user_data);
CVS_EXPORT const char *cvs_device_name(void);
CVS_EXPORT int cvs_compute_units(void);

CVS_EXPORT void *cvs_malloc(size_t bytes);
CVS_EXPORT void cvs_free(void *dev);
typedef void *cvs_graph_t;
CVS_EXPORT int cvs_graph_begin(cvs_stream_t stream);
CVS_EXPORT cvs_graph_t cvs_graph_end(cvs_stream_t stream);
CVS_EXPORT int cvs_graph_launch(cvs_graph_t graph, cvs_stream_t stream);
CVS_EXPORT void cvs_graph_destroy(cvs_graph_t graph);
CVS_EXPORT int cvs_mem_info(size_t *free_bytes, size_t *total_bytes);
CVS_EXPORT void *cvs_pool_malloc(size_t bytes, cvs_stream_t s);
CVS_EXPORT void cvs_pool_free(void *dev, cvs_stream_t s);
CVS_EXPORT void cvs_pool_trim(void);
CVS_EXPORT int cvs_memcpy_h2d(void *dev, const void *host, size_t bytes, cvs_stream_t s);
CVS_EXPORT int cvs_memcpy_d2h(void *host, const void *dev, size_t bytes, cvs_stream_t s);
CVS_EXPORT int cvs_memcpy_d2d(void *dst, const void *src, size_t bytes, cvs_stream_t s);
CVS_EXPORT int cvs_memset(void *dev, int value, size_t bytes, cvs_stream_t s);
CVS_EXPORT cvs_stream_t cvs_stream_create(void);
CVS_EXPORT void cvs_stream_destroy(cvs_stream_t s);
CVS_EXPORT int cvs_stream_sync(cvs_stream_t s);
typedef void *cvs_event_t;
CVS_EXPORT cvs_event_t cvs_event_create(void);
CVS_EXPORT void cvs_event_destroy(cvs_event_t e);
CVS_EXPORT int cvs_event_record(cvs_event_t e, cvs_stream_t s);
CVS_EXPORT int cvs_event_sync(cvs_event_t e);
CVS_EXPORT float cvs_event_elapsed_ms(cvs_event_t start, cvs_event_t stop);

CVS_EXPORT const half *cvs_lut_device(int which);
CVS_EXPORT const half *cvs_lut_host(int which);
CVS_EXPORT int cvs_lut_install(int which, const half *table_host);

CVS_EXPORT int cvs_half_to_float_dev(float *out, const half *in, size_t count, cvs_stream_t s);
CVS_EXPORT int cvs_float_to_half_dev(half *out, const float *in, size_t count, cvs_stream_t s);
CVS_EXPORT int cvs_half_to_float_fast_dev(float *out, const half *in, size_t count, cvs_stream_t s);
CVS_EXPORT int cvs_float_to_half_fast_dev(half *out, const float *in, size_t count, cvs_stream_t s);
CVS_EXPORT int cvs_half_lookup_dev(const half *table_dev, half *out, const half *in, size_t count, cvs_stream_t s);

CVS_EXPORT int cvs_frame_f16_to_f32_dev(rgba_frame_f32 *out, const rgba_frame_f16 *in, cvs_stream_t s);
CVS_EXPORT int cvs_frame_f32_to_f16_dev(rgba_frame_f16 *out, const rgba_frame_f32 *in, cvs_stream_t s);
CVS_EXPORT int cvs_copy_frame_f16_dev(rgba_frame_f16 *out, const rgba_frame_f16 *in, cvs_stream_t s);
CVS_EXPORT int cvs_copy_frame_alpha_f32_dev(rgba_frame_f32 *out, const rgba_frame_f32 *in, float alpha, cvs_stream_t s);
CVS_EXPORT int cvs_mix_cross_f32_dev(rgba_frame_f32 *out, const rgba_frame_f32 *a, const rgba_frame_f32 *b, float mix_b, cvs_stream_t s);
CVS_EXPORT int cvs_mix_over_f32_dev(rgba_frame_f32 *out, const rgba_frame_f32 *b, float mix_b, cvs_stream_t s);
CVS_EXPORT int cvs_color_matrix_f16_dev(rgba_frame_f16 *frame, const float m[9], int pre_lut, int post_lut, cvs_stream_t s);
CVS_EXPORT int cvs_color_matrix_f16_to_dev(rgba_frame_f16 *out, const rgba_frame_f16 *in, const float m[9], int pre_lut, int post_lut, cvs_stream_t s);
CVS_EXPORT int cvs_gain_offset_f16_dev(rgba_frame_f16 *out, const rgba_frame_f16 *in, float gain, float offset, cvs_stream_t s);
CVS_EXPORT int cvs_fill_solid_f16_dev(rgba_frame_f16 *frame, const box2i *window, const rgba_f32 *color, cvs_stream_t s);
CVS_EXPORT int cvs_fill_solid_f32_dev(rgba_frame_f32 *frame, const box2i *window, const rgba_f32 *color, cvs_stream_t s);
CVS_EXPORT int cvs_scale_bilinear_f16_dev(rgba_frame_f16 *target, v2f tp, const rgba_frame_f16 *source, v2f sp, v2f fac, cvs_stream_t stream);
CVS_EXPORT int cvs_scale_bilinear_f32_batch_dev(rgba_frame_f32 *const *targets, v2f target_point, const rgba_frame_f32 *const *sources, v2f source_point,
                                                v2f factors, int count, cvs_stream_t stream);
CVS_EXPORT int cvs_scale_bilinear_f16_batch_dev(rgba_frame_f16 *const *targets, v2f target_point, const rgba_frame_f16 *const *sources, v2f source_point,
                                                v2f factors, int count, cvs_stream_t stream);
CVS_EXPORT int cvs_scale_bilinear_f32_dev(rgba_frame_f32 *target, v2f target_point, const rgba_frame_f32 *source, v2f source_point, v2f factors, cvs_stream_t s);
CVS_EXPORT int cvs_fir_blur_f32_dev(rgba_frame_f32 *target, const rgba_frame_f32 *source, const float *taps_host, int ntaps, cvs_stream_t s);
#define CODED_IMAGE_MAX_PLANES 4
typedef struct {
    void *data[CODED_IMAGE_MAX_PLANES];
    int stride[CODED_IMAGE_MAX_PLANES];
    int line_count[CODED_IMAGE_MAX_PLANES];
    void (*free_func)(void *image);
} coded_image;
CVS_EXPORT coded_image *coded_image_alloc(const int *strides, const int *line_counts, int count);
CVS_EXPORT coded_image *coded_image_alloc0(const int *strides, const int *line_counts, int count);
CVS_EXPORT void video_reconstruct_dv(rgba_frame_f16 *frame, coded_image *planar);
CVS_EXPORT coded_image *video_subsample_dv(rgba_frame_f16 *frame);
CVS_EXPORT int cvs_reconstruct_dv_dev(rgba_frame_f16 *frame, const coded_image *planar, cvs_stream_t stream);
CVS_EXPORT int cvs_subsample_dv_dev(coded_image *planar, rgba_frame_f16 *frame, int encode_input_in_place, cvs_stream_t stream);
CVS_EXPORT coded_image *video_subsample_mpeg2(rgba_frame_f16 *frame);
CVS_EXPORT int cvs_subsample_mpeg2_dev(coded_image *planar, const rgba_frame_f16 *frame, int width, int height, cvs_stream_t stream);
enum { CVS_YCC_PROGRESSIVE = 1, CVS_YCC_REC709 = 2 };
CVS_EXPORT int cvs_reconstruct_mpeg2_dev(rgba_frame_f16 *frame, const coded_image *planar, int width, int height, int flags, cvs_stream_t stream);
CVS_EXPORT void video_reconstruct_mpeg2(rgba_frame_f16 *frame, coded_image *planar);

CVS_EXPORT int cvs_pulldown23_frames(int offset, int frame_index, int *first, int *second);
CVS_EXPORT int cvs_weave_fields_f16_dev(rgba_frame_f16 *frame, const rgba_frame_f16 *other, cvs_stream_t stream);

CVS_EXPORT int cvs_field_to_frame_f16_dev(rgba_frame_f16 *out, const rgba_frame_f16 *in, int field, cvs_stream_t stream);
CVS_EXPORT int cvs_soften_fields_f16_dev(rgba_frame_f16 *out, const rgba_frame_f16 *in, cvs_stream_t stream);
CVS_EXPORT int cvs_interlace_fields_f16_dev(rgba_frame_f16 *out, const rgba_frame_f16 *even, const rgba_frame_f16 *odd, cvs_stream_t stream);
CVS_EXPORT int cvs_pulldown23_add_frames(int offset, int frame_index, int *even_source, int *odd_source);

enum { CVS_DISPLAY_RGBA8 = 0, CVS_DISPLAY_ARGB32_PREMUL = 1 };
CVS_EXPORT int cvs_frame_to_bytes_dev(void *dst_dev, const rgba_frame_f16 *frame, int pre_lut, int mode, cvs_stream_t stream);
CVS_EXPORT int video_frame_to_bytes(void *dst_host, const rgba_frame_f16 *host_frame, int pre_lut, int mode);
CVS_EXPORT int cvs_frame_to_rgba8_intent_dev(void *dst_dev, const rgba_frame_f16 *frame, int pre_lut, float rendering_intent, cvs_stream_t stream);
CVS_EXPORT int video_frame_to_rgba8_intent(void *dst_host, const rgba_frame_f16 *host_frame, int pre_lut, float rendering_intent);

CVS_EXPORT int cvs_fir_blur_f16_dev(rgba_frame_f16 *target, const rgba_frame_f16 *source, const float *taps, int ntaps, cvs_stream_t stream);
CVS_EXPORT int cvs_unsharp_mask_f32_dev(rgba_frame_f32 *target, const rgba_frame_f32 *source, const float *taps, int ntaps, float amount, float threshold, cvs_stream_t s);
CVS_EXPORT int cvs_unsharp_mask_f16_dev(rgba_frame_f16 *target, const rgba_frame_f16 *source, const float *taps, int ntaps, float amount, float threshold, cvs_stream_t s);
enum { CVS_KEY_SHOW_MATTE = 1 };
typedef struct cvs_chroma_key {
    float key[3];
    float tolerance;
    float softness;
    float spill;
    float spill_range;
    int   flags;
} cvs_chroma_key;
CVS_EXPORT int cvs_chroma_key_f32_dev(rgba_frame_f32 *target, const rgba_frame_f32 *source, const cvs_chroma_key *key, cvs_stream_t s);
CVS_EXPORT int cvs_chroma_key_f16_dev(rgba_frame_f16 *target, const rgba_frame_f16 *source, const cvs_chroma_key *key, cvs_stream_t s);
CVS_EXPORT int cvs_blur_over_f16_dev(rgba_frame_f16 *out, const rgba_frame_f16 *source, const float *taps, int ntaps,
                                     const rgba_frame_f16 *const *overlays, int noverlays, cvs_stream_t stream);
CVS_EXPORT int cvs_resample_lanczos_f32_dev(rgba_frame_f32 *target, const rgba_frame_f32 *source, float factor_x, float factor_y, int kernel_size, cvs_stream_t s);
CVS_EXPORT int cvs_resample_lanczos_f16_dev(rgba_frame_f16 *target, const rgba_frame_f16 *source, float factor_x, float factor_y, int kernel_size, cvs_stream_t s);
CVS_EXPORT int cvs_blur_lanczos_f16_dev(rgba_frame_f16 *target, const rgba_frame_f16 *source, const float *taps_host, int ntaps,
                                        float factor_x, float factor_y, int kernel_size, cvs_stream_t s);
CVS_EXPORT int cvs_blur_over_f16_batch_dev(rgba_frame_f16 *const *outs, const rgba_frame_f16 *const *sources, const float *taps, int ntaps,
                                           const rgba_frame_f16 *const *overlays, int noverlays, int count, cvs_stream_t stream);
CVS_EXPORT int cvs_blur_lanczos_f16_batch_dev(rgba_frame_f16 *const *targets, const rgba_frame_f16 *const *sources, int count,
                                              const float *taps_host, int ntaps, float fx, float fy, int ksize, cvs_stream_t stream);

enum { CVS_FIR_PATH_AUTO = 0, CVS_FIR_PATH_PASSES = 1 , CVS_FIR_PATH_TILED = 2, CVS_FIR_PATH_TABLES = 4 ,
       CVS_FIR_PATH_HV = 16 ,
       CVS_FIR_PATH_ONE_COLUMN = 32 ,
       CVS_FIR_PATH_TWO_COLUMNS = 64 ,
       CVS_FIR_PATH_STRIPS = 128 ,
       CVS_FIR_PATH_TILES = 256  };
CVS_EXPORT void cvs_fir_path_override(int mode);
enum { CVS_FIR_KERNEL_NONE = 0,
       CVS_FIR_KERNEL_WINDOW = 1,
       CVS_FIR_KERNEL_HALVE = 2,
       CVS_FIR_KERNEL_VH = 4,
       CVS_FIR_KERNEL_TILED = 5,
       CVS_FIR_KERNEL_RETIRED_6 = 6,
       CVS_FIR_KERNEL_TWO_PASS = 7,
       CVS_FIR_KERNEL_PASS = 8,
       CVS_FIR_KERNEL_HV = 9,
       CVS_FIR_KERNEL_WINDOW_PAIR = 10,
       CVS_FIR_KERNEL_HALVE_PAIR = 11,
       CVS_FIR_KERNEL_TILE_VH = 12,
       CVS_FIR_KERNEL_UNSHARP = 13 };
CVS_EXPORT int cvs_fir_last_kernel(void);
CVS_EXPORT int cvs_fir_fell_through_count(void);

#define CVS_CHAIN_MAX_LAYERS 8
typedef struct {
    rgba_frame_f16 *out;
    const rgba_frame_f16 *layers[CVS_CHAIN_MAX_LAYERS];
    int nlayers;
} cvs_chain_job;
CVS_EXPORT int cvs_chain_color_over_f16_dev(const cvs_chain_job *jobs, int njobs, const float m[9],
                                            int pre_lut, int post_lut, cvs_stream_t s);
CVS_EXPORT int cvs_chain_last_was_fused(void);
CVS_EXPORT int cvs_scale_last_was_fused(void);
CVS_EXPORT int cvs_chain_last_launch_count(void);
CVS_EXPORT int cvs_mix_cross_f16_dev(rgba_frame_f16 *out, const rgba_frame_f16 *a, const rgba_frame_f16 *b, float mix_b, cvs_stream_t stream);

#if defined(__cplusplus)
}
#endif
#endif
```

Baseline: 257,200.

## Fuse colour-matrix grading into the blur+over pair kernel

Adds a fused colour-matrix + vertical/horizontal blur + alpha-over kernel that applies LUTs and the 3x3 matrix while loading source rows. The blur sweep body moves into a shared header so the plain and graded variants reuse it. The stream pipeline now calls the fused entry point and no longer allocates an intermediate graded frame. This removes one full-frame write and read of the intermediate through HBM, at the cost of extra ALU and LUT lookups inside the blur loop. Unsupported shapes fall back to the old two-kernel path through a pooled temporary.

```diff
diff --git a/canvas_amd/_lib.py b/canvas_amd/_lib.py
--- a/canvas_amd/_lib.py
+++ b/canvas_amd/_lib.py
@@ -182,6 +182,9 @@
     "cvs_resample_lanczos_f16_dev": (C.c_int, [_F16, _F16, C.c_float, C.c_float, C.c_int, _vp]),
     "cvs_blur_lanczos_f16_dev": (C.c_int, [_F16, _F16, _f32p, C.c_int, C.c_float, C.c_float, C.c_int, _vp]),
     "cvs_blur_over_f16_batch_dev": (C.c_int, [P(_F16), P(_F16), _f32p, C.c_int, P(_F16), C.c_int, C.c_int, _vp]),
+    "cvs_color_blur_over_f16_dev": (C.c_int, [_F16, _F16, _f32p, C.c_int, P(_F16), C.c_int, _f32p, C.c_int, C.c_int, _vp]),
+    "cvs_color_blur_over_f16_batch_dev": (C.c_int, [P(_F16), P(_F16), _f32p, C.c_int, P(_F16), C.c_int, C.c_int, _f32p, C.c_int, C.c_int, _vp]),
+    "cvs_color_blur_last_was_fused": (C.c_int, []),
     "cvs_scale_bilinear_f16_batch_dev": (C.c_int, [P(_F16), v2f, P(_F16), v2f, v2f, C.c_int, _vp]),
     "cvs_scale_bilinear_f32_batch_dev": (C.c_int, [P(_F32), v2f, P(_F32), v2f, v2f, C.c_int, _vp]),
     "cvs_blur_lanczos_f16_batch_dev": (C.c_int, [P(_F16), P(_F16), C.c_int, _f32p, C.c_int, C.c_float, C.c_float, C.c_int, _vp]),
diff --git a/canvas_amd/csrc/host/scale.c b/canvas_amd/csrc/host/scale.c
--- a/canvas_amd/csrc/host/scale.c
+++ b/canvas_amd/csrc/host/scale.c
@@ -713,6 +713,125 @@
     return rc;
 }
 
+
+static _Thread_local int t_color_blur_fused = -1;
+CVS_EXPORT int cvs_color_blur_last_was_fused(void) { return t_color_blur_fused; }
+
+static bool bytes_overlap(const void *a, size_t na, const void *b, size_t nb) {
+    const uintptr_t x = (uintptr_t)a, y = (uintptr_t)b;
+    return x < y + nb && y < x + na;
+}
+
+static int color_blur_fused(const any_frame *t, const any_frame *src, const box2i *win, const float m[9], const half *pre, const half *post,
+                            const float *taps, int ntaps, const void *const *over, int nover, const cvk_frame_batch *batch, hipStream_t s) {
+    if (!blur_has_fast_kernel(taps, ntaps) || ntaps > 31) return 1;
+    cvk_blur_params bp;
+    memset(&bp, 0, sizeof bp);
+    bp.nover = nover;
+    for (int l = 0; l < nover; l++) bp.over[l] = over[l];
+    bp.target = cvs_view(t->data, &t->full);
+    bp.source = cvs_view(src->data, &src->full);
+    bp.in_half = bp.out_half = 1;
+    bp.tx0 = win->min.x; bp.ty0 = win->min.y; bp.tx1 = win->max.x; bp.ty1 = win->max.y;
+    bp.sx0 = src->cur.min.x; bp.sy0 = src->cur.min.y; bp.sx1 = src->cur.max.x; bp.sy1 = src->cur.max.y;
+    bp.ntaps = ntaps;
+    memcpy(bp.taps, taps, sizeof(float) * (size_t)ntaps);
+    if (batch) bp.batch = *batch;
+    bp.flags = blur_column_pins();
+    if (!CVK(cvk_grade_blur_pair_supported)(&bp, (const uint16_t *)pre, (const uint16_t *)post)) return 1;
+    const int n = batch ? batch->n : 1;
+    for (int i = 0; i < n; i++)
+        for (int j = 0; j < n; j++)
+            if (bytes_overlap(batch ? batch->target[i] : t->data, any_bytes(t), batch ? batch->source[j] : src->data, any_bytes(src))) return 1;
+    int rc = CVK(cvk_grade_blur_pair)(&bp, m, (const uint16_t *)pre, (const uint16_t *)post, cvs_cus(), s);
+    if (rc != 0) { cvs_set_error("colour + blur launch failed: %s", hipGetErrorString((hipError_t)rc)); return -1; }
+    t_fir_kernel = CVS_FIR_KERNEL_WINDOW_PAIR;
+    return 0;
+}
+
+CVS_EXPORT int cvs_color_blur_over_f16_dev(rgba_frame_f16 *out, const rgba_frame_f16 *source, const float *taps, int ntaps,
+                                           const rgba_frame_f16 *const *overlays, int noverlays, const float m[9], int pre_lut, int post_lut,
+                                           cvs_stream_t stream) {
+    if (cvs_enter() != 0) { box2i_set_empty(&out->current_window); return -1; }
+    CVS_REQUIRE_INSIDE(source, out, "cvs_color_blur_over_f16_dev");
+    if (ntaps < 1 || !taps || !m || noverlays < 0 || (noverlays > 0 && !overlays)) { cvs_set_error("colour+blur+over: bad arguments"); box2i_set_empty(&out->current_window); return -1; }
+    const half *pre = cvs_lut_dev_or_null(pre_lut), *post = cvs_lut_dev_or_null(post_lut);
+    if ((pre_lut != CVS_LUT_NONE && !pre) || (post_lut != CVS_LUT_NONE && !post)) { box2i_set_empty(&out->current_window); return -1; }
+    hipStream_t s = cvs_pick_stream(stream);
+    const box2i *full = &out->full_window;
+    box2i win;
+    box2i_intersect(&win, &source->current_window, full);
+    bool whole = !box2i_is_empty(&win) && noverlays <= CVK_BLUR_MAX_OVER && (noverlays == 0 || same_box(&win, full));
+    const void *bufs[CVK_BLUR_MAX_OVER];
+    for (int l = 0; whole && l < noverlays; l++) {
+        whole = same_box(&overlays[l]->full_window, full) && same_box(&overlays[l]->current_window, full);
+        bufs[l] = overlays[l]->data;
+    }
+    if (whole) {
+        const any_frame o = { out->data, *full, *full, 1 }, src = { (void *)source->data, source->full_window, source->current_window, 1 };
+        const int rc = color_blur_fused(&o, &src, &win, m, pre, post, taps, ntaps, bufs, noverlays, NULL, s);
+        if (rc == 0) { out->current_window = win; t_color_blur_fused = 1; return 0; }
+        if (rc < 0) { box2i_set_empty(&out->current_window); return rc; }
+    }
+    t_color_blur_fused = 0;
+    rgba_frame_f16 graded = { NULL, source->full_window, source->full_window };
+    const size_t n = cvs_box_pixels(&graded.full_window);
+    if (n) {
+        graded.data = cvs_pool_malloc(n * sizeof(rgba_f16), s);
+        if (!graded.data) { box2i_set_empty(&out->current_window); return -1; }
+    }
+    int rc = cvs_color_matrix_f16_to_dev(&graded, source, m, pre_lut, post_lut, stream);
+    if (rc == 0) rc = cvs_blur_over_f16_dev(out, &graded, taps, ntaps, overlays, noverlays, stream);
+    else box2i_set_empty(&out->current_window);
+    cvs_pool_free(graded.data, s);
+    return rc;
+}
+
+CVS_EXPORT int cvs_color_blur_over_f16_batch_dev(rgba_frame_f16 *const *outs, const rgba_frame_f16 *const *sources, const float *taps, int ntaps,
+                                                 const rgba_frame_f16 *const *overlays, int noverlays, int count, const float m[9], int pre_lut,
+                                                 int post_lut, cvs_stream_t stream) {
+    const char *what = "cvs_color_blur_over_f16_batch_dev";
+    if (count <= 0) return 0;
+    if (ntaps < 1 || !taps || !m || noverlays < 0 || (noverlays > 0 && !overlays)) { cvs_set_error("%s: bad arguments", what); return -1; }
+    for (int i = 0; i < count; i++)
+        for (int l = 0; l < noverlays; l++)
+            if (!overlays[(size_t)i * noverlays + l]) { cvs_set_error("%s: layer %d of frame %d is a null pointer", what, l, i); return -1; }
+    if (batch_refused(outs, sources, count, 1, what)) return -1;
+    if (cvs_enter() != 0) { batch_empty_from(outs, 0, count, 1); return -1; }
+    const half *pre = cvs_lut_dev_or_null(pre_lut), *post = cvs_lut_dev_or_null(post_lut);
+    if ((pre_lut != CVS_LUT_NONE && !pre) || (post_lut != CVS_LUT_NONE && !post)) { batch_empty_from(outs, 0, count, 1); return -1; }
+    hipStream_t s = cvs_pick_stream(stream);
+    const box2i *full = &outs[0]->full_window;
+    bool uniform = count > 1 && noverlays >= 1 && noverlays <= CVK_BLUR_MAX_OVER && !box2i_is_empty(full) && (ntaps & 1);
+    for (int i = 0; uniform && i < count; i++) {
+        uniform = same_box(&outs[i]->full_window, full) && same_box(&sources[i]->full_window, &sources[0]->full_window) &&
+                  same_box(&sources[i]->current_window, full) && same_box(&sources[0]->full_window, full);
+        for (int l = 0; uniform && l < noverlays; l++) {
+            const rgba_frame_f16 *ov = overlays[(size_t)i * noverlays + l];
+            uniform = same_box(&ov->full_window, full) && same_box(&ov->current_window, full);
+        }
+    }
+    int rc = 0, done = 0, all_fused = 1;
+    const size_t bytes = cvs_box_pixels(full) * sizeof(rgba_f16);
+    while (uniform && rc == 0 && done < count) {
+        const int n = count - done < CVK_FRAME_BATCH ? count - done : CVK_FRAME_BATCH;
+        cvk_frame_batch b;
+        if (!batch_group(&b, outs, sources, 1, done, n, bytes, bytes, overlays, noverlays)) break;
+        const any_frame t = { b.target[0], *full, *full, 1 }, src = { (void *)b.source[0], sources[done]->full_window, sources[done]->current_window, 1 };
+        rc = color_blur_fused(&t, &src, full, m, pre, post, taps, ntaps, b.over[0], noverlays, &b, s);
+        if (rc == 1) { rc = 0; break; }
+        if (rc == 0) { for (int i = 0; i < n; i++) outs[done + i]->current_window = *full; done += n; }
+    }
+    for (; rc == 0 && done < count; done++) {
+        rc = cvs_color_blur_over_f16_dev(outs[done], sources[done], taps, ntaps, noverlays ? overlays + (size_t)done * noverlays : NULL, noverlays,
+                                         m, pre_lut, post_lut, stream);
+        if (t_color_blur_fused != 1) all_fused = 0;
+    }
+    if (rc != 0) batch_empty_from(outs, done, count, 1);
+    else t_color_blur_fused = all_fused;
+    return rc;
+}
+
 CVS_EXPORT int cvs_blur_lanczos_f16_batch_dev(rgba_frame_f16 *const *targets, const rgba_frame_f16 *const *sources, int count,
                                               const float *taps, int ntaps, float fx, float fy, int ksize, cvs_stream_t stream) {
     const char *what = "cvs_blur_lanczos_f16_batch_dev";
diff --git a/canvas_amd/csrc/kernels/blur_pair_ops.hip b/canvas_amd/csrc/kernels/blur_pair_ops.hip
--- a/canvas_amd/csrc/kernels/blur_pair_ops.hip
+++ b/canvas_amd/csrc/kernels/blur_pair_ops.hip
@@ -1,6 +1,6 @@
 #include <cstdlib>
 #include <atomic>
-#include "pair_common.hpp"
+#include "blur_pair_sweep.hpp"
 
 namespace {
 
@@ -8,18 +8,10 @@
 
 template <int NT, int W, int NOV>
 __global__ __launch_bounds__(W) void k_blur_pair(cvk_blur_params bp) {
-    constexpr int C = NT / 2, D = C & 1, OUTW = 2 * W - 2 * C - 2 * D, PITCH = W + 8;
     static_assert(NT & 1 && NT >= 3 && NT <= 15, "odd tap counts up to 15");
     static_assert(NOV >= 0 && NOV <= CVK_BLUR_MAX_OVER, "layer count");
-    __shared__ float4 rowbuf[2][2][PITCH];
+    __shared__ float4 rowbuf[2][2][StripGeometry<NT, W>::PITCH];
     const int lane = threadIdx.x;
-    const int xo = bp.tx0 + (int)blockIdx.x * OUTW;
-    const int sfirst = xo - C - D;
-    const int tcol = xo + 2 * lane;
-    const int ta = bp.ty0 + (int)blockIdx.y * bp.rows_per_wg;
-    const int tb = min(ta + bp.rows_per_wg - 1, bp.ty1);
-    const int ys0 = ta - C;
-    const int steps = (tb - ta) + NT;
 
     float w[NT];
 #pragma unroll
@@ -34,123 +26,12 @@
 #pragma unroll
     for (int l = 0; l < NOV; l++) over_data[l] = bp.batch.n ? ka->batch.over[z][l] : bp.over[l];
 
-    const size_t srow = (size_t)bp.source.pitch * 8, trow = (size_t)bp.target.pitch * 8;
-    const uint32_t soff = (uint32_t)((sfirst + 2 * lane - bp.sx0) * 8);
-    const uint32_t toff = 2 * lane < OUTW ? (uint32_t)((tcol - bp.tx0) * 8) : 0x80000000u;
-#ifdef CVS_DIAG
-    const uint32_t swin = (bp.flags & 0x100) ? 0u : (uint32_t)(bp.sx1 - bp.sx0 + 1) * 8u, trect = (uint32_t)(bp.tx1 - bp.tx0 + 1) * 8u;
-    const uint32_t orect = (bp.flags & 0x200) ? 0u : trect, wrect = (bp.flags & 0x400) ? 0u : trect;
-#else
-    const uint32_t swin = (uint32_t)(bp.sx1 - bp.sx0 + 1) * 8u, trect = (uint32_t)(bp.tx1 - bp.tx0 + 1) * 8u, orect = trect, wrect = trect;
-#endif
-    const char *swin0 = reinterpret_cast<const char *>(src_data) + (ptrdiff_t)(bp.sx0 - bp.source.fx0) * 8;
-    const ptrdiff_t trect0 = (ptrdiff_t)(bp.tx0 - bp.target.fx0) * 8;
-
-    if (lane < PITCH - W) {
-#pragma unroll
-        for (int b = 0; b < 2; b++)
-#pragma unroll
-            for (int ph = 0; ph < 2; ph++) rowbuf[b][ph][W + lane] = make_float4(0.f, 0.f, 0.f, 0.f);
-    }
-
-    Px ring[NT][2];
-#pragma unroll
-    for (int k = 0; k < NT; k++) ring[k][0].rg = ring[k][0].ba = ring[k][1].rg = ring[k][1].ba = f32x2{ 0.0f, 0.0f };
-
-    auto fetch_row = [&](int ys, bool wanted) {
-        const bool live = wanted && ys >= bp.sy0 && ys <= bp.sy1;
-        return load_pair(row_rsrc(swin0, (size_t)((ptrdiff_t)(ys - bp.source.fy0) * (ptrdiff_t)srow), live ? swin : 0u), soff);
-    };
-    struct Layers { u32x4 v[NOV > 0 ? NOV : 1]; };
-    auto fetch_layers = [&](int i) {
-        Layers r;
-        const bool emits = i >= NT - 1 && i < steps;
-        const size_t o = (size_t)((ptrdiff_t)(ta + i - (NT - 1) - bp.target.fy0) * (ptrdiff_t)trow + trect0);
-#pragma unroll
-        for (int l = 0; l < NOV; l++) r.v[l] = load_pair(row_rsrc(over_data[l], o, emits ? orect : 0u), toff);
-        return r;
-    };
-    u32x4 cur = fetch_row(ys0, true);
-    rowbuf[0][0][lane] = widen_px(cur.x, cur.y);
-    rowbuf[0][1][lane] = widen_px(cur.z, cur.w);
-    cur = fetch_row(ys0 + 1, steps > 1);
-    u32x4 nxt = fetch_row(ys0 + 2, steps > 2);
-    Layers ov_cur = fetch_layers(0);
-
-    for (int i0 = 0; i0 < steps; i0 += NT) {
-        auto step = [&](auto jc) -> bool {
-            constexpr int j = decltype(jc)::value;
-            const int i = i0 + j;
-            if (i >= steps) return false;
-            const bool emits = i >= NT - 1;
-            const int t = ta + (i - (NT - 1));
-            const u32x4 far = fetch_row(ys0 + i + 3, i + 3 < steps);
-            const Layers ov_nxt = fetch_layers(i + 1);
-            float4 (*buf)[PITCH] = rowbuf[i & 1];
-            __syncthreads();
-            float4 v[NT + 1];
-#pragma unroll
-            for (int c = 0; c <= NT; c++) v[c] = buf[(c + D) & 1][lane + ((c + D) >> 1)];
-            float4 (*nbuf)[PITCH] = rowbuf[(i + 1) & 1];
-            nbuf[0][lane] = widen_px(cur.x, cur.y);
-            nbuf[1][lane] = widen_px(cur.z, cur.w);
-            cur = nxt;
-            nxt = far;
-            f32x2 rg0, ba0, rg1, ba1;
-#pragma unroll
-            for (int k = 0; k < NT; k++) {
-                if constexpr (cvs::kContract) {
-                    if (k == 0) { rg0 = f32x2{ v[0].x, v[0].y } * w[0]; ba0 = f32x2{ v[0].z, v[0].w } * w[0]; rg1 = f32x2{ v[1].x, v[1].y } * w[0]; ba1 = f32x2{ v[1].z, v[1].w } * w[0]; }
-                    else {
-                        rg0 = cvs::madd(f32x2{ v[k].x, v[k].y }, w[k], rg0); ba0 = cvs::madd(f32x2{ v[k].z, v[k].w }, w[k], ba0);
-                        rg1 = cvs::madd(f32x2{ v[k + 1].x, v[k + 1].y }, w[k], rg1); ba1 = cvs::madd(f32x2{ v[k + 1].z, v[k + 1].w }, w[k], ba1);
-                    }
-                } else {
-                const f32x2 p0 = f32x2{ v[k].x, v[k].y } * w[k], q0 = f32x2{ v[k].z, v[k].w } * w[k];
-                const f32x2 p1 = f32x2{ v[k + 1].x, v[k + 1].y } * w[k], q1 = f32x2{ v[k + 1].z, v[k + 1].w } * w[k];
-                if (k == 0) { rg0 = p0; ba0 = q0; rg1 = p1; ba1 = q1; }
-                else { rg0 = rg0 + p0; ba0 = ba0 + q0; rg1 = rg1 + p1; ba1 = ba1 + q1; }
-                }
-            }
-            ring[j][0].rg = rg0; ring[j][0].ba = ba0;
-            ring[j][1].rg = rg1; ring[j][1].ba = ba1;
-            if (emits) {
-                f32x2 org0, oba0, org1, oba1;
-#pragma unroll
-                for (int k = 0; k < NT; k++) {
-                    const Px &a = ring[(j + 1 + k) % NT][0], &b = ring[(j + 1 + k) % NT][1];
-                    if constexpr (cvs::kContract) {
-                        if (k == 0) { org0 = a.rg * w[0]; oba0 = a.ba * w[0]; org1 = b.rg * w[0]; oba1 = b.ba * w[0]; }
-                        else { org0 = cvs::madd(a.rg, w[k], org0); oba0 = cvs::madd(a.ba, w[k], oba0); org1 = cvs::madd(b.rg, w[k], org1); oba1 = cvs::madd(b.ba, w[k], oba1); }
-                    } else {
-                    const f32x2 p0 = a.rg * w[k], q0 = a.ba * w[k], p1 = b.rg * w[k], q1 = b.ba * w[k];
-                    if (k == 0) { org0 = p0; oba0 = q0; org1 = p1; oba1 = q1; }
-                    else { org0 = org0 + p0; oba0 = oba0 + q0; org1 = org1 + p1; oba1 = oba1 + q1; }
-                    }
-                }
-                u32x4 codes;
-                if constexpr (NOV > 0) {
-                    cvs::px32x2 acc;
-                    acc.r = f32x2{ org0.x, org1.x }; acc.g = f32x2{ org0.y, org1.y };
-                    acc.b = f32x2{ oba0.x, oba1.x }; acc.a = f32x2{ oba0.y, oba1.y };
-#pragma unroll
-                    for (int l = 0; l < NOV; l++) acc = cvs::over_pair_uniform(acc, ov_cur.v[l]);
-                    codes = cvs::narrow_pair_lean(acc);
-                } else {
-                    codes = u32x4{ cvs::f2h_rz2(org0.x, org0.y), cvs::f2h_rz2(oba0.x, oba0.y), cvs::f2h_rz2(org1.x, org1.y), cvs::f2h_rz2(oba1.x, oba1.y) };
-                }
-                __builtin_amdgcn_raw_buffer_store_b128(codes, row_rsrc(dst_data, (size_t)((ptrdiff_t)(t - bp.target.fy0) * (ptrdiff_t)trow + trect0), wrect), (int)toff, 0, 0);
-            }
-            ov_cur = ov_nxt;
-            return true;
-        };
-        each_slot(step, std::make_integer_sequence<int, NT>{});
-    }
+    sweep_segment<NT, W, NOV>(bp, src_data, dst_data, over_data, (int)blockIdx.x, (int)blockIdx.y, rowbuf, lane, w, RowsF32{});
 }
 
 template <int NT, int W, int NOV>
 int launch(cvk_blur_params bp, int cus, hipStream_t s) {
-    constexpr int C = NT / 2, D = C & 1, OUTW = 2 * W - 2 * C - 2 * D;
+    constexpr int OUTW = StripGeometry<NT, W>::OUTW;
     const int cols = bp.tx1 - bp.tx0 + 1, rows = bp.ty1 - bp.ty0 + 1;
     const int strips = (cols + OUTW - 1) / OUTW;
     static std::atomic<int> cached{ 0 };
diff --git a/canvas_amd/csrc/kernels/blur_pair_sweep.hpp b/canvas_amd/csrc/kernels/blur_pair_sweep.hpp
--- /dev/null
+++ b/canvas_amd/csrc/kernels/blur_pair_sweep.hpp
@@ -0,0 +1,150 @@
+#pragma once
+#include "pair_common.hpp"
+
+namespace pairsweep {
+
+struct RowsF32 {
+    typedef float4 slot_t;
+    static __device__ __forceinline__ void put(slot_t &s, uint32_t lo, uint32_t hi) { s = widen_px(lo, hi); }
+    static __device__ __forceinline__ float4 get(const slot_t &s) { return s; }
+    static __device__ __forceinline__ void sync() { __syncthreads(); }
+    __device__ __forceinline__ u32x4 prepare(u32x4 v, bool, bool) const { return v; }
+};
+
+template <int NT, int W> struct StripGeometry {
+    static constexpr int C = NT / 2, D = C & 1, OUTW = 2 * W - 2 * C - 2 * D, PITCH = W + 8;
+};
+
+template <int NT, int W, int NOV, class Rows>
+__device__ __forceinline__ void sweep_segment(const cvk_blur_params &bp, const void *src_data, void *dst_data, const void *(&over_data)[NOV > 0 ? NOV : 1],
+                                              int strip, int seg, typename Rows::slot_t (*rowbuf)[2][W + 8], int lane, const float (&w)[NT], const Rows &rows) {
+    typedef StripGeometry<NT, W> G;
+    constexpr int C = G::C, D = G::D, OUTW = G::OUTW, PITCH = G::PITCH;
+    typedef typename Rows::slot_t slot_t;
+    const int xo = bp.tx0 + strip * OUTW;
+    const int sfirst = xo - C - D;
+    const int tcol = xo + 2 * lane;
+    const int ta = bp.ty0 + seg * bp.rows_per_wg;
+    const int tb = min(ta + bp.rows_per_wg - 1, bp.ty1);
+    const int ys0 = ta - C;
+    const int steps = (tb - ta) + NT;
+
+    const size_t srow = (size_t)bp.source.pitch * 8, trow = (size_t)bp.target.pitch * 8;
+    const uint32_t soff = (uint32_t)((sfirst + 2 * lane - bp.sx0) * 8);
+    const uint32_t toff = 2 * lane < OUTW ? (uint32_t)((tcol - bp.tx0) * 8) : 0x80000000u;
+#ifdef CVS_DIAG
+    const uint32_t swin = (bp.flags & 0x100) ? 0u : (uint32_t)(bp.sx1 - bp.sx0 + 1) * 8u, trect = (uint32_t)(bp.tx1 - bp.tx0 + 1) * 8u;
+    const uint32_t orect = (bp.flags & 0x200) ? 0u : trect, wrect = (bp.flags & 0x400) ? 0u : trect;
+#else
+    const uint32_t swin = (uint32_t)(bp.sx1 - bp.sx0 + 1) * 8u, trect = (uint32_t)(bp.tx1 - bp.tx0 + 1) * 8u, orect = trect, wrect = trect;
+#endif
+    const char *swin0 = reinterpret_cast<const char *>(src_data) + (ptrdiff_t)(bp.sx0 - bp.source.fx0) * 8;
+    const ptrdiff_t trect0 = (ptrdiff_t)(bp.tx0 - bp.target.fx0) * 8;
+    const bool ok = soff < swin;
+
+    if (lane < PITCH - W) {
+#pragma unroll
+        for (int b = 0; b < 2; b++)
+#pragma unroll
+            for (int ph = 0; ph < 2; ph++) Rows::put(rowbuf[b][ph][W + lane], 0u, 0u);
+    }
+
+    Px ring[NT][2];
+#pragma unroll
+    for (int k = 0; k < NT; k++) ring[k][0].rg = ring[k][0].ba = ring[k][1].rg = ring[k][1].ba = f32x2{ 0.0f, 0.0f };
+
+    auto row_live = [&](int ys, bool wanted) { return wanted && ys >= bp.sy0 && ys <= bp.sy1; };
+    auto fetch_row = [&](int ys, bool wanted) {
+        const bool live = row_live(ys, wanted);
+        return load_pair(row_rsrc(swin0, (size_t)((ptrdiff_t)(ys - bp.source.fy0) * (ptrdiff_t)srow), live ? swin : 0u), soff);
+    };
+    struct Layers { u32x4 v[NOV > 0 ? NOV : 1]; };
+    auto fetch_layers = [&](int i) {
+        Layers r;
+        const bool emits = i >= NT - 1 && i < steps;
+        const size_t o = (size_t)((ptrdiff_t)(ta + i - (NT - 1) - bp.target.fy0) * (ptrdiff_t)trow + trect0);
+#pragma unroll
+        for (int l = 0; l < NOV; l++) r.v[l] = load_pair(row_rsrc(over_data[l], o, emits ? orect : 0u), toff);
+        return r;
+    };
+    u32x4 cur = fetch_row(ys0, true);
+    cur = rows.prepare(cur, row_live(ys0, true), ok);
+    Rows::put(rowbuf[0][0][lane], cur.x, cur.y);
+    Rows::put(rowbuf[0][1][lane], cur.z, cur.w);
+    cur = fetch_row(ys0 + 1, steps > 1);
+    u32x4 nxt = fetch_row(ys0 + 2, steps > 2);
+    Layers ov_cur = fetch_layers(0);
+
+    for (int i0 = 0; i0 < steps; i0 += NT) {
+        auto step = [&](auto jc) -> bool {
+            constexpr int j = decltype(jc)::value;
+            const int i = i0 + j;
+            if (i >= steps) return false;
+            const bool emits = i >= NT - 1;
+            const int t = ta + (i - (NT - 1));
+            const u32x4 far = fetch_row(ys0 + i + 3, i + 3 < steps);
+            const Layers ov_nxt = fetch_layers(i + 1);
+            slot_t (*buf)[PITCH] = rowbuf[i & 1];
+            Rows::sync();
+            float4 v[NT + 1];
+#pragma unroll
+            for (int c = 0; c <= NT; c++) v[c] = Rows::get(buf[(c + D) & 1][lane + ((c + D) >> 1)]);
+            slot_t (*nbuf)[PITCH] = rowbuf[(i + 1) & 1];
+            cur = rows.prepare(cur, row_live(ys0 + i + 1, i + 1 < steps), ok);
+            Rows::put(nbuf[0][lane], cur.x, cur.y);
+            Rows::put(nbuf[1][lane], cur.z, cur.w);
+            cur = nxt;
+            nxt = far;
+            f32x2 rg0, ba0, rg1, ba1;
+#pragma unroll
+            for (int k = 0; k < NT; k++) {
+                if constexpr (cvs::kContract) {
+                    if (k == 0) { rg0 = f32x2{ v[0].x, v[0].y } * w[0]; ba0 = f32x2{ v[0].z, v[0].w } * w[0]; rg1 = f32x2{ v[1].x, v[1].y } * w[0]; ba1 = f32x2{ v[1].z, v[1].w } * w[0]; }
+                    else {
+                        rg0 = cvs::madd(f32x2{ v[k].x, v[k].y }, w[k], rg0); ba0 = cvs::madd(f32x2{ v[k].z, v[k].w }, w[k], ba0);
+                        rg1 = cvs::madd(f32x2{ v[k + 1].x, v[k + 1].y }, w[k], rg1); ba1 = cvs::madd(f32x2{ v[k + 1].z, v[k + 1].w }, w[k], ba1);
+                    }
+                } else {
+                const f32x2 p0 = f32x2{ v[k].x, v[k].y } * w[k], q0 = f32x2{ v[k].z, v[k].w } * w[k];
+                const f32x2 p1 = f32x2{ v[k + 1].x, v[k + 1].y } * w[k], q1 = f32x2{ v[k + 1].z, v[k + 1].w } * w[k];
+                if (k == 0) { rg0 = p0; ba0 = q0; rg1 = p1; ba1 = q1; }
+                else { rg0 = rg0 + p0; ba0 = ba0 + q0; rg1 = rg1 + p1; ba1 = ba1 + q1; }
+                }
+            }
+            ring[j][0].rg = rg0; ring[j][0].ba = ba0;
+            ring[j][1].rg = rg1; ring[j][1].ba = ba1;
+            if (emits) {
+                f32x2 org0, oba0, org1, oba1;
+#pragma unroll
+                for (int k = 0; k < NT; k++) {
+                    const Px &a = ring[(j + 1 + k) % NT][0], &b = ring[(j + 1 + k) % NT][1];
+                    if constexpr (cvs::kContract) {
+                        if (k == 0) { org0 = a.rg * w[0]; oba0 = a.ba * w[0]; org1 = b.rg * w[0]; oba1 = b.ba * w[0]; }
+                        else { org0 = cvs::madd(a.rg, w[k], org0); oba0 = cvs::madd(a.ba, w[k], oba0); org1 = cvs::madd(b.rg, w[k], org1); oba1 = cvs::madd(b.ba, w[k], oba1); }
+                    } else {
+                    const f32x2 p0 = a.rg * w[k], q0 = a.ba * w[k], p1 = b.rg * w[k], q1 = b.ba * w[k];
+                    if (k == 0) { org0 = p0; oba0 = q0; org1 = p1; oba1 = q1; }
+                    else { org0 = org0 + p0; oba0 = oba0 + q0; org1 = org1 + p1; oba1 = oba1 + q1; }
+                    }
+                }
+                u32x4 codes;
+                if constexpr (NOV > 0) {
+                    cvs::px32x2 acc;
+                    acc.r = f32x2{ org0.x, org1.x }; acc.g = f32x2{ org0.y, org1.y };
+                    acc.b = f32x2{ oba0.x, oba1.x }; acc.a = f32x2{ oba0.y, oba1.y };
+#pragma unroll
+                    for (int l = 0; l < NOV; l++) acc = cvs::over_pair_uniform(acc, ov_cur.v[l]);
+                    codes = cvs::narrow_pair_lean(acc);
+                } else {
+                    codes = u32x4{ cvs::f2h_rz2(org0.x, org0.y), cvs::f2h_rz2(oba0.x, oba0.y), cvs::f2h_rz2(org1.x, org1.y), cvs::f2h_rz2(oba1.x, oba1.y) };
+                }
+                __builtin_amdgcn_raw_buffer_store_b128(codes, row_rsrc(dst_data, (size_t)((ptrdiff_t)(t - bp.target.fy0) * (ptrdiff_t)trow + trect0), wrect), (int)toff, 0, 0);
+            }
+            ov_cur = ov_nxt;
+            return true;
+        };
+        each_slot(step, std::make_integer_sequence<int, NT>{});
+    }
+}
+
+}
diff --git a/canvas_amd/csrc/kernels/grade_blur_pair_ops.hip b/canvas_amd/csrc/kernels/grade_blur_pair_ops.hip
--- /dev/null
+++ b/canvas_amd/csrc/kernels/grade_blur_pair_ops.hip
@@ -0,0 +1,143 @@
+#include <atomic>
+#include "blur_pair_sweep.hpp"
+#include "lut_common.hpp"
+#include "grade.hpp"
+
+namespace {
+
+using namespace pairsweep;
+using cvs::kLutHalfs;
+
+constexpr int kWave = 64;
+constexpr int waves_for(int nt, int nov) { return (nt >= 13 || (nt >= 11 && nov >= 1)) ? 8 : 12; }
+
+template <bool PRE, bool POST>
+struct RowsGraded {
+    typedef uint2 slot_t;
+    const cvs::MatR &mat;
+    const uint16_t *lut, *post;
+    static __device__ __forceinline__ void put(slot_t &s, uint32_t lo, uint32_t hi) { s = make_uint2(lo, hi); }
+    static __device__ __forceinline__ float4 get(const slot_t &s) { const uint2 p = s; return widen_px(p.x, p.y); }
+    static __device__ __forceinline__ void sync() {
+        __builtin_amdgcn_fence(__ATOMIC_RELEASE, "wavefront");
+        __builtin_amdgcn_wave_barrier();
+        __builtin_amdgcn_fence(__ATOMIC_ACQUIRE, "wavefront");
+    }
+    __device__ __forceinline__ u32x4 prepare(u32x4 v, bool live, bool ok) const {
+        if (!live) return u32x4{ 0u, 0u, 0u, 0u };
+        const u32x4 g = cvs::color_pair_codes<PRE, POST>(v, mat, lut, post);
+        return ok ? g : u32x4{ 0u, 0u, 0u, 0u };
+    }
+};
+
+template <int NT, int NOV, bool PRE, bool POST, int NW>
+__global__ __launch_bounds__(NW * kWave) void k_grade_blur_pair(cvk_blur_params bp, cvs::Mat kmat, const uint16_t *__restrict__ pre,
+                                                                const uint16_t *__restrict__ post, int strips, int segs, int items) {
+    static_assert(NT & 1 && NT >= 3 && NT <= 13, "odd tap counts up to 13");
+    static_assert(NOV >= 0 && NOV <= CVK_BLUR_MAX_OVER, "layer count");
+    static_assert(PRE || POST, "a kernel without a table has no reason to be one workgroup per CU");
+    constexpr int PITCH = StripGeometry<NT, kWave>::PITCH;
+    __shared__ uint16_t lut[kLutHalfs];
+    __shared__ uint2 rowbuf[NW][2][2][PITCH];
+    const cvs::MatR mat = CVS_MAT_REGS(kmat);
+    const int wave = __builtin_amdgcn_readfirstlane((int)threadIdx.x / kWave), lane = (int)threadIdx.x % kWave;
+
+    {
+        const uint4 *src = reinterpret_cast<const uint4 *>(PRE ? pre : post);
+        uint4 *dst = reinterpret_cast<uint4 *>(lut);
+        constexpr int kWords = kLutHalfs * 2 / 16, kPer = (kWords + NW * kWave - 1) / (NW * kWave);
+        const int rot = (int)(blockIdx.x >> 3);
+        for (int it = 0; it < kPer; it++) {
+            const int i = ((it + rot) % kPer) * (NW * kWave) + (int)threadIdx.x;
+            if (i < kWords) dst[i] = src[i];
+        }
+        __syncthreads();
+    }
+
+    float w[NT];
+#pragma unroll
+    for (int k = 0; k < NT; k++) w[k] = bp.taps[k];
+    typedef const cvk_blur_params __attribute__((address_space(4))) *kargs_t;
+    const kargs_t ka = (kargs_t)__builtin_amdgcn_kernarg_segment_ptr();
+    const RowsGraded<PRE, POST> rows{ mat, lut, post };
+
+    for (int item = (int)blockIdx.x * NW + wave; item < items; item += (int)gridDim.x * NW) {
+        const int strip = item % strips, rest = item / strips, seg = rest % segs, z = rest / segs;
+        const void *src_data = bp.batch.n ? ka->batch.source[z] : bp.source.data;
+        void *dst_data = bp.batch.n ? ka->batch.target[z] : bp.target.data;
+        const void *over_data[NOV > 0 ? NOV : 1];
+#pragma unroll
+        for (int l = 0; l < NOV; l++) over_data[l] = bp.batch.n ? ka->batch.over[z][l] : bp.over[l];
+        sweep_segment<NT, kWave, NOV>(bp, src_data, dst_data, over_data, strip, seg, rowbuf[wave], lane, w, rows);
+    }
+}
+
+template <int NT, int NOV, bool PRE, bool POST>
+int launch(cvk_blur_params bp, const cvs::Mat &mat, const uint16_t *pre, const uint16_t *post, int cus, hipStream_t s) {
+    constexpr int NW = waves_for(NT, NOV), OUTW = StripGeometry<NT, kWave>::OUTW;
+    const int cols = bp.tx1 - bp.tx0 + 1, rows = bp.ty1 - bp.ty0 + 1;
+    const int strips = (cols + OUTW - 1) / OUTW;
+    const int nframes = bp.batch.n > 0 ? bp.batch.n : 1;
+    const int wgs = cus > 0 ? cus : 256;
+    if (bp.rows_per_wg <= 0) {
+        int segs = (NW * wgs) / (strips * nframes);
+        if (segs < 1) segs = 1;
+        int r = (rows + segs - 1) / segs;
+        if (r < NT - 1) r = NT - 1;
+        if (r > rows) r = rows;
+        bp.rows_per_wg = r;
+    }
+    const int segs = (rows + bp.rows_per_wg - 1) / bp.rows_per_wg;
+    const int items = strips * segs * nframes;
+    int grid = (items + NW - 1) / NW;
+    if (grid > wgs) grid = wgs;
+    hipLaunchKernelGGL((k_grade_blur_pair<NT, NOV, PRE, POST, NW>), dim3((unsigned)grid), dim3(NW * kWave), 0, s, bp, mat, pre, post, strips, segs, items);
+    return (int)hipGetLastError();
+}
+
+template <int NT, int NOV>
+int pick_tables(const cvk_blur_params *bp, const cvs::Mat &mat, const uint16_t *pre, const uint16_t *post, int cus, hipStream_t s) {
+    if (pre && post) return launch<NT, NOV, true, true>(*bp, mat, pre, post, cus, s);
+    if (pre) return launch<NT, NOV, true, false>(*bp, mat, pre, post, cus, s);
+    return launch<NT, NOV, false, true>(*bp, mat, pre, post, cus, s);
+}
+
+template <int NT>
+int pick_layers(const cvk_blur_params *bp, const cvs::Mat &mat, const uint16_t *pre, const uint16_t *post, int cus, hipStream_t s) {
+    switch (bp->nover) {
+    case 0: return pick_tables<NT, 0>(bp, mat, pre, post, cus, s);
+    case 1: return pick_tables<NT, 1>(bp, mat, pre, post, cus, s);
+    case 2: return pick_tables<NT, 2>(bp, mat, pre, post, cus, s);
+    case 3: return pick_tables<NT, 3>(bp, mat, pre, post, cus, s);
+    case 4: return pick_tables<NT, 4>(bp, mat, pre, post, cus, s);
+    }
+    return (int)hipErrorInvalidValue;
+}
+
+}
+
+extern "C" int cvk_grade_blur_pair_supported(const cvk_blur_params *bp, const uint16_t *pre, const uint16_t *post) {
+    if (!pre && !post) return 0;
+    if (!aligned16(pre) || !aligned16(post)) return 0;
+    if (bp->step != 0 && bp->step != 1) return 0;
+    return cvk_blur_takes_pairs(bp);
+}
+
+extern "C" int cvk_grade_blur_pair(const cvk_blur_params *bp_in, const float m[9], const uint16_t *pre, const uint16_t *post, int cus, void *stream) {
+    if (bp_in->tx1 < bp_in->tx0 || bp_in->ty1 < bp_in->ty0) return 0;
+    if (!cvk_grade_blur_pair_supported(bp_in, pre, post)) return (int)hipErrorInvalidValue;
+    cvk_blur_params bp = *bp_in;
+    bp.step = 1;
+    bp.flags = 0;
+    const cvs::Mat mat = cvs::make_mat(m);
+    hipStream_t s = (hipStream_t)stream;
+    switch (bp.ntaps) {
+    case 3: return pick_layers<3>(&bp, mat, pre, post, cus, s);
+    case 5: return pick_layers<5>(&bp, mat, pre, post, cus, s);
+    case 7: return pick_layers<7>(&bp, mat, pre, post, cus, s);
+    case 9: return pick_layers<9>(&bp, mat, pre, post, cus, s);
+    case 11: return pick_layers<11>(&bp, mat, pre, post, cus, s);
+    case 13: return pick_layers<13>(&bp, mat, pre, post, cus, s);
+    }
+    return (int)hipErrorInvalidValue;
+}
diff --git a/canvas_amd/csrc/kernels/kernels.h b/canvas_amd/csrc/kernels/kernels.h
--- a/canvas_amd/csrc/kernels/kernels.h
+++ b/canvas_amd/csrc/kernels/kernels.h
@@ -32,6 +32,8 @@
 #define cvk_blur                     cvk_blur_fma
 #define cvk_blur_pair_supported      cvk_blur_pair_supported_fma
 #define cvk_blur_pair                cvk_blur_pair_fma
+#define cvk_grade_blur_pair_supported cvk_grade_blur_pair_supported_fma
+#define cvk_grade_blur_pair          cvk_grade_blur_pair_fma
 #define cvk_blur_halve_pair_supported cvk_blur_halve_pair_supported_fma
 #define cvk_blur_halve_pair          cvk_blur_halve_pair_fma
 #define cvk_blur_halve_supported     cvk_blur_halve_supported_fma
@@ -190,6 +192,8 @@
 int cvk_blur_takes_pairs(const cvk_blur_params *bp);
 int cvk_blur_pair_supported(const cvk_blur_params *bp);
 int cvk_blur_pair(const cvk_blur_params *bp, int cus, void *stream);
+int cvk_grade_blur_pair_supported(const cvk_blur_params *bp, const uint16_t *pre_lut, const uint16_t *post_lut);
+int cvk_grade_blur_pair(const cvk_blur_params *bp, const float m[9], const uint16_t *pre_lut, const uint16_t *post_lut, int cus, void *stream);
 
 typedef struct {
     cvk_view target, source;
@@ -266,6 +270,8 @@
 int cvk_blur_fma(const cvk_blur_params *bp, int cus, void *stream);
 int cvk_blur_pair_supported_fma(const cvk_blur_params *bp);
 int cvk_blur_pair_fma(const cvk_blur_params *bp, int cus, void *stream);
+int cvk_grade_blur_pair_supported_fma(const cvk_blur_params *bp, const uint16_t *pre_lut, const uint16_t *post_lut);
+int cvk_grade_blur_pair_fma(const cvk_blur_params *bp, const float m[9], const uint16_t *pre_lut, const uint16_t *post_lut, int cus, void *stream);
 int cvk_blur_halve_pair_supported_fma(const cvk_blur_halve_params *bp);
 int cvk_blur_halve_pair_fma(const cvk_blur_halve_params *bp, int cus, void *stream);
 int cvk_blur_halve_supported_fma(int ntaps1, int ntaps2);
diff --git a/canvas_amd/stream.py b/canvas_amd/stream.py
--- a/canvas_amd/stream.py
+++ b/canvas_amd/stream.py
@@ -7,7 +7,7 @@
 from .shard import frames_of_rank
 
 NODE_BYTES_PER_PIXEL = 16 + 16 + 40
-BYTES_PER_PIXEL = 16 + 40
+BYTES_PER_PIXEL = 40
 OVERLAYS = 3
 
 
@@ -38,8 +38,7 @@
                 frames.append(d)
             src, over = frames[0], frames[1:]
             refs = (C.POINTER(_lib.rgba_frame_f16_t) * overlays)(*[C.pointer(o.c) for o in over])
-            self.slots.append({"src": src, "over": over, "over_refs": refs, "graded": DeviceFrame(self.full, np.uint16),
-                               "out": DeviceFrame(self.full, np.uint16)})
+            self.slots.append({"src": src, "over": over, "over_refs": refs, "out": DeviceFrame(self.full, np.uint16)})
         _lib.check(self.lib.cvs_stream_sync(None), "donor copies")
         self._m = self.matrix.ctypes.data_as(C.POINTER(C.c_float))
         self._t = self.taps.ctypes.data_as(C.POINTER(C.c_float))
@@ -50,24 +49,22 @@
 
     def render(self, slot, stream=None):
         s, lib = self.slots[slot % self.ring], self.lib
-        _lib.check(lib.cvs_color_matrix_f16_to_dev(s["graded"].ref(), s["src"].ref(), self._m, self.pre_lut, self.post_lut, stream), "colour")
-        _lib.check(lib.cvs_blur_over_f16_dev(s["out"].ref(), s["graded"].ref(), self._t, len(self.taps), s["over_refs"],
-                                             self.overlays, stream), "blur+over")
+        _lib.check(lib.cvs_color_blur_over_f16_dev(s["out"].ref(), s["src"].ref(), self._t, len(self.taps), s["over_refs"], self.overlays,
+                                                   self._m, self.pre_lut, self.post_lut, stream), "colour+blur+over")
         return s["out"]
 
     def render_batch(self, slots, stream=None):
         lib, n = self.lib, len(slots)
         ss = [self.slots[i % self.ring] for i in slots]
-        for s in ss:
-            _lib.check(lib.cvs_color_matrix_f16_to_dev(s["graded"].ref(), s["src"].ref(), self._m, self.pre_lut, self.post_lut, stream), "colour")
         key = tuple(i % self.ring for i in slots)
         if getattr(self, "_batch_key", None) != key:
             fp = C.POINTER(_lib.rgba_frame_f16_t)
             self._b_out = (fp * n)(*[C.pointer(s["out"].c) for s in ss])
-            self._b_src = (fp * n)(*[C.pointer(s["graded"].c) for s in ss])
+            self._b_src = (fp * n)(*[C.pointer(s["src"].c) for s in ss])
             self._b_ov = (fp * (n * self.overlays))(*[C.pointer(o.c) for s in ss for o in s["over"]])
             self._batch_key = key
-        _lib.check(lib.cvs_blur_over_f16_batch_dev(self._b_out, self._b_src, self._t, len(self.taps), self._b_ov, self.overlays, n, stream), "blur+over batch")
+        _lib.check(lib.cvs_color_blur_over_f16_batch_dev(self._b_out, self._b_src, self._t, len(self.taps), self._b_ov, self.overlays, n,
+                                                         self._m, self.pre_lut, self.post_lut, stream), "colour+blur+over batch")
         return [s["out"] for s in ss]
 
     def run(self, frames_per_rank, rank=0, world=1, stream=None):
diff --git a/include/canvas_hip.h b/include/canvas_hip.h
--- a/include/canvas_hip.h
+++ b/include/canvas_hip.h
@@ -302,6 +302,13 @@
                                            const rgba_frame_f16 *const *overlays, int noverlays, int count, cvs_stream_t stream);
 CVS_EXPORT int cvs_blur_lanczos_f16_batch_dev(rgba_frame_f16 *const *targets, const rgba_frame_f16 *const *sources, int count,
                                               const float *taps_host, int ntaps, float fx, float fy, int ksize, cvs_stream_t stream);
+CVS_EXPORT int cvs_color_blur_over_f16_dev(rgba_frame_f16 *out, const rgba_frame_f16 *source, const float *taps, int ntaps,
+                                           const rgba_frame_f16 *const *overlays, int noverlays, const float m[9], int pre_lut, int post_lut,
+                                           cvs_stream_t stream);
+CVS_EXPORT int cvs_color_blur_over_f16_batch_dev(rgba_frame_f16 *const *outs, const rgba_frame_f16 *const *sources, const float *taps, int ntaps,
+                                                 const rgba_frame_f16 *const *overlays, int noverlays, int count, const float m[9], int pre_lut,
+                                                 int post_lut, cvs_stream_t stream);
+CVS_EXPORT int cvs_color_blur_last_was_fused(void);
 
 enum { CVS_FIR_PATH_AUTO = 0, CVS_FIR_PATH_PASSES = 1 , CVS_FIR_PATH_TILED = 2, CVS_FIR_PATH_TABLES = 4 ,
        CVS_FIR_PATH_HV = 16 ,
```

Result: no change. 256,900 (-0.1%).
